# elizabethfong/SparkSmithWaterman

Hardware: AMD Instinct MI355X
Metric: GCUPS (higher is better)
Workload: dtype int32

## Files before the change

sparksmithwaterman_amd/csrc/swmi_api.cpp:

```cpp
#include <hip/hip_runtime.h>

#include <algorithm>
#include <atomic>
#include <chrono>
#include <condition_variable>
#include <unistd.h>
#include <cstdarg>
#include <cstdio>
#include <cstdlib>
#include <cstring>
#include <memory>
#include <mutex>
#include <numeric>
#include <string>
#include <thread>
#include <unordered_map>
#include <deque>
#include <vector>

#include "../../include/swmi.h"
#include "swmi_device.h"
#include "swmi_io_internal.h"

extern "C" hipError_t swmi_launch_fill(const FillArgs *a, hipStream_t st, hipEvent_t ev_start, hipEvent_t ev_stop);
extern "C" hipError_t swmi_launch_traceback(const TraceArgs *a, hipStream_t st, hipEvent_t ev_start, hipEvent_t ev_stop);
extern "C" hipError_t swmi_launch_traceback_split(const TraceArgs *a, uint32_t n_windows, hipStream_t st);
extern "C" hipError_t swmi_launch_resident(const TraceArgs *a, const ResidentArgs *x, hipStream_t st);
extern "C" hipError_t swmi_launch_tfused(const TraceArgs *a, const TFusedArgs *x, hipStream_t st);
extern "C" hipError_t swmi_launch_affine_sweep(const FillArgs *a, int32_t gap_open, uint32_t r_min, uint32_t r_max, hipStream_t st);
extern "C" hipError_t swmi_launch_affine_traceback(const TraceArgs *a, uint32_t tile_words, uint32_t ops_words, hipStream_t st);
extern "C" hipError_t swmi_launch_encode(const uint8_t *raw, const uint64_t *raw_off, SeqDesc *desc, uint32_t *seqw,
                                         const uint8_t *lut, uint32_t n_seq, hipStream_t st);

static thread_local std::string g_err;

static int fail(int code, const char *fmt, ...) {
    char buf[512];
    va_list ap;
    va_start(ap, fmt);
    vsnprintf(buf, sizeof buf, fmt, ap);
    va_end(ap);
    g_err = buf;
    return code;
}

int swmi_io_fail(int code, const std::string &msg) { return fail(code, "%s", msg.c_str()); }

#define HIP_TRY(expr)                                                                         \
    do {                                                                                      \
        hipError_t e_ = (expr);                                                               \
        if (e_ != hipSuccess)                                                                 \
            return fail(e_ == hipErrorOutOfMemory ? SWMI_ERR_NOMEM : SWMI_ERR_HIP,            \
                        "%s failed: %s", #expr, hipGetErrorString(e_));                       \
    } while (0)

struct DevBuf {
    void *p = nullptr;
    size_t cap = 0;
    int reserve(size_t bytes) {
        if (bytes <= cap) return SWMI_OK;
        size_t want = bytes >= (256u << 20) ? bytes + bytes / 2 : bytes;
        if (p) { want = std::max(want, cap + cap / 4); (void)hipFree(p); p = nullptr; cap = 0; }
        hipError_t e = hipMalloc(&p, want);
        if (e != hipSuccess && want > bytes) { want = bytes; e = hipMalloc(&p, want); }
        if (e != hipSuccess) { p = nullptr; return fail(SWMI_ERR_NOMEM, "hipMalloc(%zu) failed: %s", bytes, hipGetErrorString(e)); }
        cap = want;
        return SWMI_OK;
    }
    void release() { if (p) (void)hipFree(p); p = nullptr; cap = 0; }
    template <class T> T *as() const { return (T *)p; }
    DevBuf() = default;
    DevBuf(const DevBuf &) = delete;
    DevBuf &operator=(const DevBuf &) = delete;
    ~DevBuf() { release(); }
};

struct PinnedBuf {
    void *p = nullptr;
    void *dp = nullptr;
    size_t cap = 0;
    int reserve(size_t bytes) {
        if (bytes <= cap) return SWMI_OK;
        if (p) { bytes = std::max(bytes, cap + cap / 4); (void)hipHostFree(p); p = nullptr; dp = nullptr; cap = 0; }
        hipError_t e = hipHostMalloc(&p, bytes, hipHostMallocMapped);
        if (e != hipSuccess) { p = nullptr; return fail(SWMI_ERR_NOMEM, "hipHostMalloc(%zu) failed: %s", bytes, hipGetErrorString(e)); }
        e = hipHostGetDevicePointer(&dp, p, 0);
        if (e != hipSuccess) { (void)hipHostFree(p); p = nullptr; return fail(SWMI_ERR_HIP, "hipHostGetDevicePointer: %s", hipGetErrorString(e)); }
        cap = bytes;
        return SWMI_OK;
    }
    void release() { if (p) (void)hipHostFree(p); p = nullptr; dp = nullptr; cap = 0; }
    PinnedBuf() = default;
    PinnedBuf(const PinnedBuf &) = delete;
    PinnedBuf &operator=(const PinnedBuf &) = delete;
    ~PinnedBuf() { release(); }
};

struct swmi_ctx {
    int device = 0;
    hipStream_t stream = nullptr;
    std::mutex mu;
    uint32_t cell_cap = 64;
    uint64_t max_workspace_bytes = 32ull << 30;
    int profiling = 0;
    uint32_t mode = 1;
    int zero_copy = 1;
    uint64_t arena_words_per_pair = 160;
    uint64_t arena_copy_wpp = 160;
    uint64_t recs_per_pair_x16 = 32;
    hipEvent_t ev[6] = {nullptr, nullptr, nullptr, nullptr, nullptr, nullptr};
    PinnedBuf h_err;
    DevBuf d_hdr_ring;
    uint32_t hdr_next = 0;
    DevBuf d_lut;
    int64_t spin_us = 2000;
    uint32_t dbg_strip_spins = 0;
    uint32_t dbg_reverse_strips = 0;
    uint32_t auto_ties_x100 = 300;
    uint32_t col_chunks = 0;
    int tb_split = -1;
    bool ext_events = false;
    int tfused = -1;
    int resident = -1;
    int scores_only = 0;
    int stream_keep_records = 1;
    int device_strings = 1;
    bool cell_cap_set = false;
    int32_t gap_open = 0;
    int affine = -1;
    std::thread worker;
    std::mutex job_mu;
    std::condition_variable job_cv;
    std::atomic<int> job_state{0};
    swmi_batch *job_batch = nullptr;
    swmi_params job_params{};
    int job_rc = 0;
    std::string job_err;
};

struct HostAln {
    uint32_t rank;
    int32_t begin, end_i, end_j;
    uint32_t n_ops;
    const uint32_t *rec = nullptr;
    int64_t str_id = -1;
};

struct PairRes {
    int32_t score = 0;
    uint32_t flags = 0;
    uint64_t n_cells = 0;
    uint64_t first = 0;
    uint64_t count = 0;
};

struct SiteRef { uint64_t pair; uint64_t k; int32_t begin; };

struct Work {
    uint32_t pair;
    uint64_t cells;
    uint64_t dir_words;
    uint64_t seam_words;
};

struct swmi_batch {
    uint32_t n_refs = 0, n_reads = 0;
    std::vector<uint8_t> ref_bytes, read_bytes;
    const uint8_t *src_map = nullptr;
    std::vector<swmi_io_recpos> src_recs;
    std::unordered_map<uint32_t, std::vector<uint8_t>> src_cache;
    std::vector<uint64_t> ref_off, read_off;
    std::vector<SeqDesc> ref_desc, read_desc;
    DevBuf d_raw, d_raw_off;
    DevBuf d_seqw, d_refs, d_reads, d_pairs, d_dir, d_seam, d_result, d_cells, d_cells_off, d_cells_cap, d_dbg, d_dbg2;
    DevBuf d_strip_items, d_progress;
    DevBuf d_col_items;
    DevBuf d_win_off, d_queue;
    DevBuf d_tf_items;
    DevBuf d_res_items;
    bool views_built = false;
    bool tb_split_used = false;
    bool acgt_known = false;
    PinnedBuf h_result;
    swmi_params params{};
    bool has_run = false;
    int auto_choice = -1;
    swmi_params auto_params{};
    std::vector<Work> work;
    int work_mode = -1;
    bool work_tfused = false;
    uint32_t eff_mode = 1;
    int32_t gap_open = 0;
    uint64_t work_cells = 0;
    std::vector<uint8_t> pairs_on_device;
    const void *pairs_dev_ptr = nullptr;
    struct Prep {
        bool valid = false;
        size_t lo = 0, hi = 0;
        const void *work = nullptr;
        swmi_params params{};
        int mode = -1;
        uint64_t dir_words = 0, seam_words = 0;
        uint32_t max_path = 0, max_read = 0;
        size_t n_strip_items = 0, n_col_items = 0, n_strip_chunks = 0;
        uint64_t n_windows = 0, seam_priv_words = 0;
        size_t n_res = 0;
        uint32_t res_lds_words = 0, res_ops_words = 0;
        int resident_opt = -1;
        int tfused_opt = -1;
        uint32_t aff_r_min = 0, aff_r_max = 0;
        size_t n_tf = 0;
        uint32_t tf_max_m = 0, tf_max_n = 0, tf_max_path = 0;
        bool exact = false, scores_only = false;
        uint32_t col_chunks_opt = 0;
        bool reverse_strips = false;
    } prep;
    std::vector<PairRes> pairs;
    struct RawChunk { size_t at, words; size_t tab_at, n_rec; size_t lo; std::vector<uint32_t> wpos; };
    std::vector<uint32_t> raw;
    std::vector<AlnRec> rtab;
    const uint32_t *raw_ext = nullptr;
    const AlnRec *rtab_ext = nullptr;
    uint64_t raw_ext_records = 0, raw_ext_cap = 0;
    std::vector<RawChunk> raw_chunks;
    bool indexed = false;
    bool rec_strings = false;
    bool scores_only = false;
    bool records_dropped = false;
    std::vector<HostAln> alns;
    std::vector<char> str_buf;
    std::vector<uint64_t> str_at;
    std::vector<int8_t> ref_view_ready;
    std::vector<std::vector<SiteRef>> ref_sites;
    std::vector<uint64_t> ref_degenerate;
    swmi_timing timing{};
};

static const uint8_t *code_table();

extern "C" int swmi_abi_version(void) { return SWMI_ABI_VERSION; }

extern "C" const char *swmi_last_error(void) { return g_err.c_str(); }

extern "C" int swmi_device_count(int *count) {
    if (!count) return fail(SWMI_ERR_INVALID, "count is null");
    int n = 0;
    hipError_t e = hipGetDeviceCount(&n);
    if (e != hipSuccess) { *count = 0; return fail(SWMI_ERR_NO_DEVICE, "hipGetDeviceCount: %s", hipGetErrorString(e)); }
    *count = n;
    return SWMI_OK;
}

extern "C" void swmi_default_params(swmi_params *p) {
    if (!p) return;
    p->match = 5; p->mismatch = -3; p->gap = -4;
    p->tie_mode = SWMI_TIE_SERIAL;
    p->types[0] = 'a'; p->types[1] = 'i'; p->types[2] = 'd'; p->types[3] = '-';
}

static void ctx_release(swmi_ctx *c) {
    for (auto &ev : c->ev) if (ev) (void)hipEventDestroy(ev);
    if (c->stream) (void)hipStreamDestroy(c->stream);
    c->h_err.release();
    c->d_lut.release();
    c->d_hdr_ring.release();
    delete c;
}

extern "C" int swmi_create(int device, swmi_ctx **out) {
    if (!out) return fail(SWMI_ERR_INVALID, "out is null");
    *out = nullptr;
    int n = 0;
    hipError_t e = hipGetDeviceCount(&n);
    if (e != hipSuccess || n <= 0)
        return fail(SWMI_ERR_NO_DEVICE, "no HIP device available (%s); this library has no CPU fallback",
                    e != hipSuccess ? hipGetErrorString(e) : "device count 0");
    if (device < 0 || device >= n) return fail(SWMI_ERR_INVALID, "device %d out of range [0,%d)", device, n);
    hipDeviceProp_t prop;
    e = hipGetDeviceProperties(&prop, device);
    if (e != hipSuccess) return fail(SWMI_ERR_NO_DEVICE, "hipGetDeviceProperties: %s", hipGetErrorString(e));
    if (strncmp(prop.gcnArchName, "gfx950", 6) != 0)
        return fail(SWMI_ERR_NO_DEVICE, "device %d is %s; the kernels are built for gfx950 (MI355X) only",
                    device, prop.gcnArchName);
    e = hipSetDevice(device);
    if (e != hipSuccess) return fail(SWMI_ERR_NO_DEVICE, "hipSetDevice: %s", hipGetErrorString(e));
    swmi_ctx *c = new swmi_ctx;
    c->device = device;
    e = hipStreamCreateWithFlags(&c->stream, hipStreamNonBlocking);
    if (e != hipSuccess) { c->stream = nullptr; ctx_release(c); return fail(SWMI_ERR_HIP, "hipStreamCreate: %s", hipGetErrorString(e)); }
    for (auto &ev : c->ev) {
        e = hipEventCreate(&ev);
        if (e != hipSuccess) { ev = nullptr; ctx_release(c); return fail(SWMI_ERR_HIP, "hipEventCreate: %s", hipGetErrorString(e)); }
    }
    { int r = c->h_err.reserve(64); if (r) { ctx_release(c); return r; } }
    { static const char *ee = getenv("SWMI_EXT_EVENTS"); if (ee) c->ext_events = atoi(ee) != 0; }
// ... 50 lines not shown
        if (value < -1 || value > 1) return fail(SWMI_ERR_INVALID, "resident must be -1 (automatic), 0 or 1");
        ctx->resident = (int)value;
    } else if (!strcmp(name, "scores_only")) {
        ctx->scores_only = value != 0;
    } else if (!strcmp(name, "stream_keep_records")) {
        ctx->stream_keep_records = value != 0;
    } else if (!strcmp(name, "device_strings")) {
        ctx->device_strings = value != 0;
    } else if (!strcmp(name, "tb_split")) {
        if (value < -1 || value > 1) return fail(SWMI_ERR_INVALID, "tb_split must be -1 (automatic), 0 or 1");
        ctx->tb_split = (int)value;
    } else if (!strcmp(name, "col_chunks")) {
        if (value < 0 || value > 4096) return fail(SWMI_ERR_INVALID, "col_chunks out of range");
        ctx->col_chunks = (uint32_t)value;
    } else if (!strcmp(name, "zero_copy")) {
        ctx->zero_copy = value != 0;
    } else if (!strcmp(name, "profiling")) {
        if (value < 0 || value > 2) return fail(SWMI_ERR_INVALID, "profiling must be 0, 1 (every stage) or 2 (the sweep only)");
        ctx->profiling = (int)value;
    } else if (!strcmp(name, "gap_open")) {
        if (value > 0) return fail(SWMI_ERR_INVALID, "gap_open must be <= 0 (a penalty), got %lld", (long long)value);
        if (value < INT32_MIN) return fail(SWMI_ERR_INVALID, "gap_open out of range");
        ctx->gap_open = (int32_t)value;
    } else if (!strcmp(name, "affine")) {
        if (value != -1 && value != 1) return fail(SWMI_ERR_INVALID, "affine must be -1 (when gap_open != 0) or 1 (always)");
        ctx->affine = (int)value;
    } else if (!strcmp(name, "arena_words_per_pair")) {
        if (value < 1) return fail(SWMI_ERR_INVALID, "arena_words_per_pair out of range");
        ctx->arena_words_per_pair = (uint64_t)value;
    } else {
        return fail(SWMI_ERR_INVALID, "unknown option '%s'", name);
    }
    return SWMI_OK;
}

static const uint8_t *code_table() {
    static uint8_t T[256];
    static std::once_flag once;
    std::call_once(once, [] {
        uint8_t perm[256];
        for (int i = 0; i < 256; i++) perm[i] = (uint8_t)i;
        const uint8_t fast[8] = {'A', 'C', 'G', 'T', 'N', 'U', 'R', 'Y'};
        for (int k = 0; k < 8; k++) std::swap(perm[fast[k]], perm[4 * k]);
        for (int i = 0; i < 256; i++) {
            int u = i;
            if ((i >= 'a' && i <= 'z') || (i >= 0xE0 && i <= 0xFE && i != 0xF7)) u = i - 32;
            T[i] = perm[u];
        }
    });
    return T;
}

static uint64_t layout_sequences(const uint64_t *off, uint32_t n, uint64_t word0, std::vector<SeqDesc> &desc) {
    desc.resize(n);
    uint64_t at = word0;
    for (uint32_t s = 0; s < n; s++) {
        const uint64_t len = off[s + 1] - off[s];
        at = (at + 3) & ~(uint64_t)3;
        SeqDesc d{};
        d.len = (uint32_t)len;
        d.boff = (uint32_t)at;
        d.acgt = 0;
        desc[s] = d;
        at += (len + 3) / 4 + SWMI_SEQ_PAD_WORDS;
    }
    return at;
}

static int check_offsets(const uint64_t *off, uint32_t n, const char *what) {
    if (!off) return fail(SWMI_ERR_INVALID, "%s offsets are null", what);
    if (off[0] != 0) return fail(SWMI_ERR_INVALID, "%s offsets must start at 0", what);
    for (uint32_t k = 0; k < n; k++) {
        if (off[k + 1] < off[k]) return fail(SWMI_ERR_INVALID, "%s offsets decrease at %u", what, k);
        if (off[k + 1] - off[k] >= (1ull << 30))
            return fail(SWMI_ERR_UNSUPPORTED, "%s %u is longer than 2^30-1 bases", what, k);
    }
    return SWMI_OK;
}

extern "C" void swmi_batch_free(swmi_ctx *ctx, swmi_batch *b) {
    if (!b) return;
    if (ctx) (void)hipSetDevice(ctx->device);
    b->d_raw.release(); b->d_raw_off.release();
    b->d_seqw.release(); b->d_refs.release(); b->d_reads.release(); b->d_pairs.release();
    b->d_dir.release(); b->d_seam.release(); b->d_result.release(); b->d_cells.release();
    b->d_cells_off.release(); b->d_cells_cap.release(); b->d_dbg.release(); b->d_dbg2.release();
    b->d_strip_items.release(); b->d_progress.release(); b->d_col_items.release(); b->d_win_off.release(); b->d_queue.release(); b->d_res_items.release();
    b->d_tf_items.release();
    b->h_result.release();
    delete b;
}

static int upload_device(swmi_ctx *ctx, swmi_batch *b, hipStream_t st, const uint8_t *ref_src, const uint8_t *read_src) {
    const uint32_t n_refs = b->n_refs, n_reads = b->n_reads;
    const uint64_t ref_total = b->ref_off[n_refs], read_total = b->read_off[n_reads];
    uint64_t words = layout_sequences(b->ref_off.data(), n_refs, 0, b->ref_desc);
    words = layout_sequences(b->read_off.data(), n_reads, words, b->read_desc);
    words = ((words + 3) & ~(uint64_t)3) + SWMI_SEQ_PAD_WORDS;
    if (words >= (1ull << 32)) return fail(SWMI_ERR_UNSUPPORTED, "sequence image exceeds 16 GiB");
    int rc;
    const uint64_t read_base = (ref_total + 15) & ~(uint64_t)15;
    if ((rc = b->d_seqw.reserve(words * 4))) return rc;
    if ((rc = b->d_raw.reserve(read_base + read_total + 16))) return rc;
    if ((rc = b->d_raw_off.reserve(((uint64_t)n_refs + n_reads + 2) * 8))) return rc;
    if ((rc = b->d_refs.reserve(std::max<size_t>(n_refs, 1) * sizeof(SeqDesc)))) return rc;
    if ((rc = b->d_reads.reserve(std::max<size_t>(n_reads, 1) * sizeof(SeqDesc)))) return rc;
    HIP_TRY(hipMemsetAsync(b->d_seqw.p, 0, words * 4, st));
    uint8_t *raw = b->d_raw.as<uint8_t>();
    uint64_t *roff = b->d_raw_off.as<uint64_t>();
    if (ref_total) HIP_TRY(hipMemcpyAsync(raw, ref_src, ref_total, hipMemcpyHostToDevice, st));
    if (read_total) HIP_TRY(hipMemcpyAsync(raw + read_base, read_src, read_total, hipMemcpyHostToDevice, st));
    HIP_TRY(hipMemcpyAsync(roff, b->ref_off.data(), ((size_t)n_refs + 1) * 8, hipMemcpyHostToDevice, st));
    std::vector<uint64_t> read_abs(b->read_off);
    for (auto &o : read_abs) o += read_base;
    HIP_TRY(hipMemcpyAsync(roff + n_refs + 1, read_abs.data(), ((size_t)n_reads + 1) * 8, hipMemcpyHostToDevice, st));
    if (n_refs) HIP_TRY(hipMemcpyAsync(b->d_refs.p, b->ref_desc.data(), n_refs * sizeof(SeqDesc), hipMemcpyHostToDevice, st));
    if (n_reads) HIP_TRY(hipMemcpyAsync(b->d_reads.p, b->read_desc.data(), n_reads * sizeof(SeqDesc), hipMemcpyHostToDevice, st));
    HIP_TRY(swmi_launch_encode(raw, roff, b->d_refs.as<SeqDesc>(), b->d_seqw.as<uint32_t>(), ctx->d_lut.as<uint8_t>(), n_refs, st));
    HIP_TRY(swmi_launch_encode(raw, roff + n_refs + 1, b->d_reads.as<SeqDesc>(), b->d_seqw.as<uint32_t>(),
                               ctx->d_lut.as<uint8_t>(), n_reads, st));
    HIP_TRY(hipStreamSynchronize(st));
    b->work_mode = -1; b->prep.valid = false; b->pairs_dev_ptr = nullptr; b->pairs_on_device.clear();
    b->has_run = false; b->acgt_known = false; b->auto_choice = -1;
    return SWMI_OK;
}

extern "C" int swmi_batch_upload(swmi_ctx *ctx,
                                 const uint8_t *ref_bytes, const uint64_t *ref_off, uint32_t n_refs,
                                 const uint8_t *read_bytes, const uint64_t *read_off, uint32_t n_reads,
                                 swmi_batch **out) {
    if (!ctx || !out) return fail(SWMI_ERR_INVALID, "null argument");
    *out = nullptr;
    int rc;
    if ((rc = check_offsets(ref_off, n_refs, "reference"))) return rc;
    if ((rc = check_offsets(read_off, n_reads, "read"))) return rc;
    if ((n_refs && ref_off[n_refs] && !ref_bytes) || (n_reads && read_off[n_reads] && !read_bytes))
        return fail(SWMI_ERR_INVALID, "sequence bytes are null");
    if ((uint64_t)n_refs * n_reads >= (1ull << 32))
        return fail(SWMI_ERR_UNSUPPORTED, "more than 2^32-1 pairs in one batch");
    std::lock_guard<std::mutex> g(ctx->mu);
    HIP_TRY(hipSetDevice(ctx->device));

    std::unique_ptr<swmi_batch> b(new swmi_batch);
    b->n_refs = n_refs; b->n_reads = n_reads;
    b->ref_off.assign(ref_off, ref_off + n_refs + 1);
    b->read_off.assign(read_off, read_off + n_reads + 1);
    b->ref_bytes.assign(ref_bytes, ref_bytes + ref_off[n_refs]);
    b->read_bytes.assign(read_bytes, read_bytes + read_off[n_reads]);
    if ((rc = upload_device(ctx, b.get(), ctx->stream, ref_bytes, read_bytes))) { swmi_batch_free(ctx, b.release()); return rc; }
    *out = b.release();
    return SWMI_OK;
}

namespace {

struct RunState {
    swmi_ctx *ctx;
    swmi_batch *b;
    FillArgs fa{};
    TraceArgs ta{};
    float fill_ms = 0, tb_ms = 0, d2h_ms = 0;
    uint32_t launches = 0;
    double enqueue_us = 0, wait_us = 0, copyout_us = 0, prep_us = 0, prep_upload_us = 0;
    bool one_wave_sweep = false;
    bool tb_split = false;
    bool defer_copy = false;
    bool keep = true;
};

inline size_t result_out_off() { return 64; }
inline size_t result_tab_off(size_t np) { return (64 + np * sizeof(PairOut) + 255) & ~(size_t)255; }
inline size_t result_arena_off(size_t np, uint64_t tab_cap) { return (result_tab_off(np) + tab_cap * sizeof(AlnRec) + 255) & ~(size_t)255; }
inline uint64_t rec_words(uint32_t n_ops, bool strings) {
    return strings ? 2 * ((uint64_t)n_ops / 4 + 1) : ((uint64_t)n_ops + 15) / 16;
}

}

#define SWMI_RES_CELL_CAP 128u

static uint64_t path_bound(uint64_t n_, uint64_t m_, const swmi_params &p) {
    uint64_t path = n_ + m_;
    if (p.match > 0 && p.gap < 0 && p.mismatch <= p.match) {
        const uint64_t g = (uint64_t)(-(int64_t)p.gap), mt = (uint64_t)p.match;
        path = std::min(path, std::min(m_ + std::min(n_, mt * m_ / g), n_ + std::min(m_, mt * n_ / g)));
    }
    return path;
}

static uint64_t traceback_lds_bytes(uint32_t mode, uint64_t max_path, uint64_t max_read) {
    const uint64_t lds_words = (max_path + 3) / 4 + 1, lds_read_words = (max_read + 3) / 4 + 1;
    const uint64_t win = (uint64_t)SWMI_RMAX * 64;
    const uint64_t tile_words = mode == 0 ? 4ull * 16 * win : (mode == 1 ? 32 + 8ull * SWMI_CK_BLOCKS * win : 4ull * SWMI_CK_BLOCKS * win);
    return 4ull * (tile_words + 4ull * (lds_words + lds_read_words + 96));
}

static int prepare_chunk(RunState &rs, const std::vector<Work> &work, size_t lo, size_t hi, const std::vector<uint64_t> *cells_exact) {
    swmi_ctx *ctx = rs.ctx;
    swmi_batch *b = rs.b;
    const size_t np = hi - lo;
    const uint32_t n_reads = b->n_reads;
    int rc;

    std::vector<PairDesc> pd;
    std::vector<StripItem> strip_items;
    uint64_t seam_priv_words = 0;
    size_t n_strip_chunks = 0;
    std::vector<ColItem> col_items;
    uint64_t dir_words = 0, seam_words = 0;
    uint32_t max_path = 0, max_read = 0;
    size_t n_strip_items = 0, n_col_items = 0;
    uint64_t n_windows = 0;
    std::vector<uint32_t> win_off;
    std::vector<uint32_t> res_items;
    size_t n_res = 0;
    uint32_t res_lds_words = 0, res_ops_words = 0;
    std::vector<uint32_t> tf_items;
    size_t n_tf = 0;
    uint32_t tf_max_m = 0, tf_max_n = 0, tf_max_path = 0;
    uint32_t aff_r_min = 0xFFFFFFFFu, aff_r_max = 0;
    const uint32_t res_cell_cap = SWMI_RES_CELL_CAP;
    swmi_batch::Prep &pr = b->prep;
    const auto p0 = std::chrono::steady_clock::now();
    const bool prepared = pr.valid && pr.lo == lo && pr.hi == hi && pr.work == (const void *)work.data() && pr.mode == b->eff_mode &&
                          memcmp(&pr.params, &b->params, sizeof(swmi_params)) == 0 && b->pairs_dev_ptr == b->d_pairs.p &&
                          b->pairs_on_device.size() == np * sizeof(PairDesc) && pr.col_chunks_opt == ctx->col_chunks &&
                          pr.reverse_strips == (ctx->dbg_reverse_strips != 0) && pr.resident_opt == ctx->resident &&
                          pr.tfused_opt == ctx->tfused && pr.exact == (cells_exact != nullptr) && pr.scores_only == (ctx->scores_only != 0);
    if (prepared) {
        dir_words = pr.dir_words; seam_words = pr.seam_words; max_path = pr.max_path; max_read = pr.max_read;
        n_strip_items = pr.n_strip_items; n_col_items = pr.n_col_items; n_windows = pr.n_windows;
        seam_priv_words = pr.seam_priv_words; n_strip_chunks = pr.n_strip_chunks;
        n_res = pr.n_res; res_lds_words = pr.res_lds_words; res_ops_words = pr.res_ops_words;
        n_tf = pr.n_tf; tf_max_m = pr.tf_max_m; tf_max_n = pr.tf_max_n; tf_max_path = pr.tf_max_path;
        aff_r_min = pr.aff_r_min; aff_r_max = pr.aff_r_max;
    } else {
    const swmi_params &P = b->params;
    const bool cols_possible = b->eff_mode == 1 && P.match > 0 && P.gap < 0 && P.mismatch <= 0 &&
                               P.match <= 7 && P.mismatch >= -8 && (np <= 512 || ctx->col_chunks > 1) && ctx->col_chunks != 1;
    const bool res_possible = b->eff_mode == 1 && !cells_exact && !ctx->scores_only && ctx->resident != 0 && (ctx->resident == 1 || np >= 256) &&
                              P.match <= 7 && P.match >= -8 && P.mismatch >= -8 && P.mismatch <= 0 && P.gap <= 0;
    auto res_need_words = [&](uint32_t m_, uint32_t n_, uint32_t &opw) -> uint64_t {
        const uint32_t R_ = swmi_rows_per_lane(m_), lact = (m_ + R_ - 1) / R_;
        const uint64_t nblk = ((uint64_t)n_ + lact - 1 + 15) / 16, n_ck = (nblk + SWMI_CK_BLOCKS - 1) / SWMI_CK_BLOCKS;
        opw = (uint32_t)((path_bound(n_, m_, P) + 15) / 16 + 1);
        return nblk * R_ * 64 + ((n_ck + 1) & ~1ull) + 2ull * res_cell_cap + 64ull * opw + (n_ + 3) / 4 + 1 + (m_ + 3) / 4 + 1 + 8 +
               128;
    };
    bool res_maybe = false;
    if (res_possible)
        for (size_t k = 0; k < np && !res_maybe; k++) {
            const uint32_t m_ = b->read_desc[work[lo + k].pair % n_reads].len, n_ = b->ref_desc[work[lo + k].pair / n_reads].len;
            uint32_t opw;
            res_maybe = m_ <= 64u * SWMI_RMAX && (ctx->resident == 1 || (uint64_t)n_ <= 8ull * m_) &&
                        res_need_words(m_, n_, opw) * 4 <= (ctx->resident == 1 ? 40u : 20u) * 1024u;
        }
    const bool tf_possible = b->eff_mode == 1 && !cells_exact && !ctx->scores_only && ctx->tfused == 1 &&
                             P.match > 0 && P.match <= 7 && P.mismatch >= -8 && P.mismatch <= P.match && P.gap < 0 && P.gap >= -64;
    if ((cols_possible || res_maybe || tf_possible) && !b->acgt_known) {
        if (b->n_refs) HIP_TRY(hipMemcpy(b->ref_desc.data(), b->d_refs.p, b->n_refs * sizeof(SeqDesc), hipMemcpyDeviceToHost));
        if (b->n_reads) HIP_TRY(hipMemcpy(b->read_desc.data(), b->d_reads.p, b->n_reads * sizeof(SeqDesc), hipMemcpyDeviceToHost));
        b->acgt_known = true;
    }
    const uint64_t chunk_budget = ctx->col_chunks > 1 ? ctx->col_chunks : std::max<uint64_t>(1, 1024 / std::max<size_t>(np, 1));
    pd.resize(np);
    if (b->eff_mode == 1) win_off.resize(np + 1);
    uint32_t pb_m = 0xFFFFFFFFu, pb_n = 0xFFFFFFFFu, pb_val = 0;
    for (size_t k = 0; k < np; k++) {
        const Work &w = work[lo + k];
        PairDesc d{};
        d.ref_id = w.pair / n_reads;
        d.read_id = w.pair % n_reads;
        d.out_id = (uint32_t)k;
        const uint32_t m_ = b->read_desc[d.read_id].len, n_ = b->ref_desc[d.ref_id].len;
        if (b->eff_mode == 1) {
            const uint64_t rps = 64ull * swmi_rows_per_lane(m_);
            const uint64_t wb = ((uint64_t)n_ + 63u + 15u) / 16u;
            win_off[k] = (uint32_t)std::min<uint64_t>(n_windows, 0xFFFFFFFFu);
            n_windows += ((m_ + rps - 1) / rps) * ((wb + SWMI_CK_BLOCKS - 1u) / SWMI_CK_BLOCKS);
        }
        uint32_t res_opw = 0;
        const bool res_fit = res_maybe && m_ <= 64u * SWMI_RMAX && b->read_desc[d.read_id].acgt && b->ref_desc[d.ref_id].acgt &&
                             (ctx->resident == 1 || (uint64_t)n_ <= 8ull * m_) &&
                             res_need_words(m_, n_, res_opw) * 4 <= (ctx->resident == 1 ? 40u : 20u) * 1024u;
        const bool tf_fit = !res_fit && tf_possible && m_ <= SWMI_TF_MAX_M && n_ <= 64u * SWMI_TF_BMAX &&
                            b->read_desc[d.read_id].acgt && b->ref_desc[d.ref_id].acgt && w.dir_words >= swmi_tf_ck_words(m_);
        if (tf_fit) {
            d.pad = SWMI_PAD_RESIDENT;
            tf_items.push_back((uint32_t)k);
            tf_max_m = std::max(tf_max_m, m_); tf_max_n = std::max(tf_max_n, n_);
            tf_max_path = std::max<uint32_t>(tf_max_path, (uint32_t)path_bound(n_, m_, P));
        } else if (res_fit) {
            d.pad = SWMI_PAD_RESIDENT;
            res_items.push_back((uint32_t)k);
            uint32_t opw;
            res_lds_words = std::max<uint32_t>(res_lds_words, (uint32_t)res_need_words(m_, n_, opw));
            res_ops_words = std::max(res_ops_words, opw);
        } else if (b->eff_mode == 1 && m_ > 64u * SWMI_RMAX && strip_items.size() < (1u << 30)) {
            const uint32_t strips = (m_ + 64u * SWMI_RMAX - 1u) / (64u * SWMI_RMAX);
            d.pad = (uint32_t)strip_items.size();
            auto push_strips = [&](StripItem it) {
                it.pair = (uint32_t)k;
                it.prog = (uint32_t)strip_items.size();
                it.pad = 0;
                if (ctx->dbg_reverse_strips) for (uint32_t st = strips; st-- > 0;) { it.strip = st; strip_items.push_back(it); }
                else                         for (uint32_t st = 0; st < strips; st++) { it.strip = st; strip_items.push_back(it); }
            };
            uint64_t chunks = 1;
            const uint64_t wblocks = ((uint64_t)n_ + 63u + 15u) / 16u;
            const uint32_t n_ck = (uint32_t)((wblocks + SWMI_CK_BLOCKS - 1u) / SWMI_CK_BLOCKS);
            const uint32_t step_w = 16u * SWMI_CK_BLOCKS;
            const uint64_t span = (uint64_t)m_ + (uint64_t)(P.match > 0 ? P.match : 0) * m_ / (uint64_t)(P.gap < 0 ? -(int64_t)P.gap : 1) + 1;
            if (cols_possible) {
                const uint64_t budget = ctx->col_chunks > 1 ? ctx->col_chunks : chunk_budget / strips;
                chunks = std::min<uint64_t>(budget, n_ / std::max<uint64_t>((span + 64) / 4, 256));
                chunks = std::min<uint64_t>(chunks, n_ck);
                if (chunks < 2) chunks = 1;
            }
            if (chunks == 1) {
                StripItem it{};
                it.col0 = 0; it.g_lo = 0; it.g_hi = 0xFFFFFFFFu; it.priv_stride = 0; it.priv_off = 0;
                push_strips(it);
            } else {
                const uint32_t wpc = (uint32_t)((n_ck + chunks - 1) / chunks);
                for (uint32_t g_lo = 0; g_lo < n_ck; g_lo += wpc) {
                    StripItem it{};
                    it.g_lo = g_lo;
                    it.g_hi = std::min(g_lo + wpc, n_ck);
                    if (it.g_hi < n_ck && (uint64_t)it.g_hi * step_w > n_) it.g_hi = n_ck;
                    const int64_t c0 = (int64_t)g_lo * step_w - 64 - (int64_t)span - 1;
                    it.col0 = g_lo == 0 || c0 <= 0 ? 0u : (uint32_t)(c0 / step_w * step_w);
                    const uint64_t ext0 = (uint64_t)it.g_hi * step_w - it.col0 + 64ull * (strips - 1u);
                    const uint64_t n0 = it.g_hi < n_ck ? std::min<uint64_t>(n_ - it.col0, ext0) : n_ - it.col0;
                    it.priv_stride = (uint32_t)((n0 + 1 + 15) & ~15ull);
                    it.priv_off = seam_priv_words;
                    seam_priv_words += (uint64_t)(strips - 1u) * it.priv_stride;
                    if (it.g_hi == n_ck) it.g_hi = 0xFFFFFFFFu;
                    push_strips(it);
                    n_strip_chunks++;
                    if (it.g_hi == 0xFFFFFFFFu) break;
                }
            }
        } else if (cols_possible && chunk_budget > 1 && m_ <= 64u * SWMI_RMAX && b->read_desc[d.read_id].acgt && b->ref_desc[d.ref_id].acgt) {
            const uint64_t span = (uint64_t)m_ + (uint64_t)P.match * m_ / (uint64_t)(-(int64_t)P.gap) + 1;
            const uint64_t wblocks = ((uint64_t)n_ + 63u + 15u) / 16u;
            const uint32_t n_ck = (uint32_t)((wblocks + SWMI_CK_BLOCKS - 1u) / SWMI_CK_BLOCKS);
            const uint32_t step_w = 16u * SWMI_CK_BLOCKS;
            uint64_t chunks = std::min<uint64_t>(chunk_budget, n_ / std::max<uint64_t>(span + 64, 256));
            chunks = std::min<uint64_t>(chunks, n_ck);
            static const bool dbg_one = getenv("SWMI_DEBUG_ONE_CHUNK") != nullptr;
            if (dbg_one) chunks = 1;
            if (chunks >= 2 || dbg_one) {
                const uint32_t wpc = (uint32_t)((n_ck + chunks - 1) / chunks);
                const size_t first = col_items.size();
                for (uint32_t g_lo = 0; g_lo < n_ck; g_lo += wpc) {
                    ColItem ci;
                    ci.pair = (uint32_t)k;
                    ci.g_lo = g_lo;
                    ci.g_hi = std::min(g_lo + wpc, n_ck);
                    if (ci.g_hi < n_ck && (uint64_t)ci.g_hi * step_w > n_) ci.g_hi = n_ck;
                    const int64_t c0 = (int64_t)g_lo * step_w - 64 - (int64_t)span - 1;
                    ci.col0 = g_lo == 0 || c0 <= 0 ? 0u : (uint32_t)(c0 / step_w * step_w);
                    col_items.push_back(ci);
                    if (ci.g_hi == n_ck) break;
                }
                d.pad = SWMI_PAD_COLS | (uint32_t)(col_items.size() - first);
            }
        }
        pd[k] = d;
        if (m_ != pb_m || n_ != pb_n) { pb_m = m_; pb_n = n_; pb_val = (uint32_t)path_bound(n_, m_, b->params); }
        max_path = std::max<uint32_t>(max_path, pb_val);
        max_read = std::max(max_read, m_);
        aff_r_min = std::min(aff_r_min, swmi_aff_rows_per_lane(m_));
        aff_r_max = std::max(aff_r_max, swmi_aff_rows_per_lane(m_));
    }
    n_strip_items = strip_items.size();
    n_col_items = col_items.size();
    n_res = res_items.size();
    n_tf = tf_items.size();
    res_lds_words = 0;
    for (uint32_t k : res_items) {
        uint32_t opw;
        const uint32_t m_ = b->read_desc[pd[k].read_id].len, n_ = b->ref_desc[pd[k].ref_id].len;
        const uint64_t own = res_need_words(m_, n_, opw);
        res_lds_words = std::max<uint32_t>(res_lds_words, (uint32_t)(own + 64ull * (res_ops_words - opw)));
    }
    if (16ull * res_lds_words > 160ull * 1024) {
        for (uint32_t k : res_items) pd[k].pad = 0;
        res_items.clear();
        n_res = 0; res_lds_words = 0; res_ops_words = 0;
    }
    {
        std::vector<uint8_t> is_res(np, 0);
        for (uint32_t k : res_items) is_res[k] = 1;
        for (size_t k = 0; k < np; k++) {
            pd[k].dir_off = dir_words;
            pd[k].seam_off = seam_words;
            if (!is_res[k]) { dir_words += work[lo + k].dir_words; seam_words += work[lo + k].seam_words; }
        }
    }
    if (b->eff_mode == 1) win_off[np] = (uint32_t)std::min<uint64_t>(n_windows, 0xFFFFFFFFu);
    for (StripItem &it : strip_items)
        if (it.priv_stride) it.priv_off += seam_words;
    }
    const auto p1 = std::chrono::steady_clock::now();
    if (!prepared && b->eff_mode == 1) {
        if ((rc = b->d_win_off.reserve((np + 1) * sizeof(uint32_t)))) return rc;
        HIP_TRY(hipMemcpyAsync(b->d_win_off.p, win_off.data(), (np + 1) * sizeof(uint32_t), hipMemcpyHostToDevice, ctx->stream));
        HIP_TRY(hipStreamSynchronize(ctx->stream));
    }
    if ((rc = b->d_pairs.reserve(np * sizeof(PairDesc)))) return rc;
    if (!prepared && !strip_items.empty()) {
        if ((rc = b->d_strip_items.reserve(strip_items.size() * sizeof(StripItem)))) return rc;
        if ((rc = b->d_progress.reserve(strip_items.size() * sizeof(uint32_t)))) return rc;
        HIP_TRY(hipMemcpyAsync(b->d_strip_items.p, strip_items.data(), strip_items.size() * sizeof(StripItem), hipMemcpyHostToDevice, ctx->stream));
        HIP_TRY(hipStreamSynchronize(ctx->stream));
    }
    if (!prepared && !res_items.empty()) {
        if ((rc = b->d_res_items.reserve(res_items.size() * sizeof(uint32_t)))) return rc;
        HIP_TRY(hipMemcpyAsync(b->d_res_items.p, res_items.data(), res_items.size() * sizeof(uint32_t), hipMemcpyHostToDevice, ctx->stream));
        HIP_TRY(hipStreamSynchronize(ctx->stream));
    }
    if (!prepared && !tf_items.empty()) {
        if ((rc = b->d_tf_items.reserve(tf_items.size() * sizeof(uint32_t)))) return rc;
        HIP_TRY(hipMemcpyAsync(b->d_tf_items.p, tf_items.data(), tf_items.size() * sizeof(uint32_t), hipMemcpyHostToDevice, ctx->stream));
        HIP_TRY(hipStreamSynchronize(ctx->stream));
    }
    if (!prepared && !col_items.empty()) {
        if ((rc = b->d_col_items.reserve(col_items.size() * sizeof(ColItem)))) return rc;
        HIP_TRY(hipMemcpyAsync(b->d_col_items.p, col_items.data(), col_items.size() * sizeof(ColItem), hipMemcpyHostToDevice, ctx->stream));
        HIP_TRY(hipStreamSynchronize(ctx->stream));
    }
    if ((rc = b->d_dir.reserve(std::max<uint64_t>(dir_words, 1) * 4))) return rc;
    if ((rc = b->d_seam.reserve(std::max<uint64_t>(seam_words + seam_priv_words, 1) * 4))) return rc;
    if (!prepared && (b->pairs_dev_ptr != b->d_pairs.p || b->pairs_on_device.size() != np * sizeof(PairDesc) ||
        memcmp(b->pairs_on_device.data(), pd.data(), np * sizeof(PairDesc)) != 0)) {
        HIP_TRY(hipMemcpyAsync(b->d_pairs.p, pd.data(), np * sizeof(PairDesc), hipMemcpyHostToDevice, ctx->stream));
        HIP_TRY(hipStreamSynchronize(ctx->stream));
        b->pairs_on_device.assign((const uint8_t *)pd.data(), (const uint8_t *)pd.data() + np * sizeof(PairDesc));
        b->pairs_dev_ptr = b->d_pairs.p;
    }
    if (!prepared) {
        pr.valid = b->pairs_dev_ptr == b->d_pairs.p;
        pr.lo = lo; pr.hi = hi; pr.work = (const void *)work.data(); pr.params = b->params; pr.mode = b->eff_mode;
        pr.dir_words = dir_words; pr.seam_words = seam_words; pr.max_path = max_path; pr.max_read = max_read;
        pr.n_strip_items = n_strip_items; pr.n_col_items = n_col_items; pr.n_windows = n_windows;
        pr.seam_priv_words = seam_priv_words; pr.n_strip_chunks = n_strip_chunks;
        pr.n_res = n_res; pr.res_lds_words = res_lds_words; pr.res_ops_words = res_ops_words;
        pr.resident_opt = ctx->resident; pr.exact = cells_exact != nullptr;
        pr.tfused_opt = ctx->tfused; pr.n_tf = n_tf; pr.tf_max_m = tf_max_m; pr.tf_max_n = tf_max_n; pr.tf_max_path = tf_max_path;
        pr.col_chunks_opt = ctx->col_chunks; pr.reverse_strips = ctx->dbg_reverse_strips != 0;
        pr.scores_only = ctx->scores_only != 0;
        pr.aff_r_min = aff_r_min; pr.aff_r_max = aff_r_max;
    }
    rs.prep_us += std::chrono::duration<double, std::micro>(p1 - p0).count();
    rs.prep_upload_us += std::chrono::duration<double, std::micro>(std::chrono::steady_clock::now() - p1).count();
    return SWMI_OK;
}

static int dump_traceback_diagnostics(swmi_batch *b, const TraceArgs &ta, size_t np, size_t n_tf) {
    if (!ta.dbg) return SWMI_OK;
    std::vector<unsigned long long> d(np * 4);
    HIP_TRY(hipMemcpy(d.data(), ta.dbg, np * 32, hipMemcpyDeviceToHost));
    if (n_tf) {
        double t0 = 0, t1 = 0, t2 = 0, t3 = 0, t4 = 0, t5 = 0; unsigned long long mx = 0;
        for (size_t k = 0; k < np; k++) {
            t0 += d[4*k]; t1 += d[4*k+1] & 0xFFFFFFFFull; t2 += d[4*k+1] >> 32; t3 += d[4*k+2] >> 16; t4 += d[4*k+3] >> 32; t5 += d[4*k+3] & 0xFFFFFFFFull;
            mx = std::max(mx, d[4*k]);
        }
        fprintf(stderr, "[swmi tfused dbg] ticks per sweeper wavefront: lifetime mean=%.0f max=%llu = prologue %.0f + sweep %.0f + first block task %.0f (%.2f block tasks per wavefront) + waiting for tasks %.0f + rest (more tasks, walk items) %.0f\n",
                t0 / np, mx, t2 / np, t1 / np, t3 / np, t5 / np, t4 / np, (t0 - t1 - t2 - t3 - t4) / np);
        {
            std::vector<size_t> idx(np);
            for (size_t k = 0; k < np; k++) idx[k] = k;
            std::sort(idx.begin(), idx.end(), [&](size_t x, size_t y) { return d[4 * x] < d[4 * y]; });
            auto at = [&](double q) { return d[4 * idx[std::min<size_t>(np - 1, (size_t)(q * np))]]; };
            fprintf(stderr, "[swmi tfused dbg]   lifetime p10=%llu p50=%llu p90=%llu p99=%llu max=%llu\n", at(0.10), at(0.50), at(0.90), at(0.99), d[4 * idx[np - 1]]);
            for (size_t t = 0; t < std::min<size_t>(np, 6); t++) {
                const size_t k = idx[np - 1 - t];
                fprintf(stderr, "[swmi tfused dbg]   slow wavefront (pair %zu): lifetime %llu, sweep %llu, first block task %llu, block tasks taken %llu, waiting %llu, alignments of its pair %llu\n",
                        k, d[4 * k], d[4 * k + 1] & 0xFFFFFFFFull, d[4 * k + 2] >> 16, d[4 * k + 3] & 0xFFFFFFFFull, d[4 * k + 3] >> 32,
                        (unsigned long long)((const PairOut *)((const uint8_t *)b->h_result.p + result_out_off()))[k].n_cells);
            }
        }
    }
    double a0 = 0, a1 = 0, a2 = 0, a3 = 0; unsigned long long mx = 0;
    double a4 = 0;
    for (size_t k = 0; k < np; k++) { a0 += d[4*k]; a1 += d[4*k+1] & 0xFFFFFFFFull; a2 += d[4*k+2] & 0xFFFF; a4 += d[4*k+2] >> 16; a3 += d[4*k+3] & 0xFFFFFFFFull; mx = std::max(mx, d[4*k]); }
    fprintf(stderr, "[swmi tb dbg] wave ticks mean=%.0f max=%llu; walk ticks mean=%.0f; staging ticks mean=%.0f; steps mean=%.1f; iterations mean=%.2f\n",
            a0 / np, mx, a1 / np, a4 / np, a2 / np, a3 / np);
    const PairOut *po_dbg = (const PairOut *)((const uint8_t *)b->h_result.p + result_out_off());
    double cs[4] = {0, 0, 0, 0}, cw[4] = {0, 0, 0, 0}; unsigned long long cm[4] = {0, 0, 0, 0}; size_t cn[4] = {0, 0, 0, 0};
    for (size_t k = 0; k < np; k++) {
        const size_t c = std::min<uint64_t>(po_dbg[k].n_cells, 4) - (po_dbg[k].n_cells ? 1 : 0);
        cs[c] += d[4 * k]; cw[c] += d[4 * k + 1] & 0xFFFFFFFFull; cm[c] = std::max(cm[c], d[4 * k]); cn[c]++;
    }
    {
        std::vector<size_t> idx(np);
        for (size_t k = 0; k < np; k++) idx[k] = k;
        const size_t top = std::min<size_t>(np, 6);
        std::partial_sort(idx.begin(), idx.begin() + top, idx.end(), [&](size_t x, size_t y) { return d[4 * x] > d[4 * y]; });
        for (size_t t = 0; t < top; t++)
            fprintf(stderr, "[swmi tb dbg]   slow pair %zu: ticks=%llu walk=%llu staging=%llu in %llu stagings, steps=%llu iterations=%llu alignments=%llu\n", idx[t],
                    d[4 * idx[t]], d[4 * idx[t] + 1] & 0xFFFFFFFFull, d[4 * idx[t] + 2] >> 16, d[4 * idx[t] + 3] >> 32, d[4 * idx[t] + 2] & 0xFFFF,
                    d[4 * idx[t] + 3] & 0xFFFFFFFFull, (unsigned long long)po_dbg[idx[t]].n_cells);
        for (size_t t = 0; t < top; t++)
            fprintf(stderr, "[swmi tb dbg]     ... of the staging time of pair %zu, %llu ticks waiting for helpers\n", idx[t], d[4 * idx[t] + 1] >> 32);
    }
    for (int c = 0; c < 4; c++)
        if (cn[c]) fprintf(stderr, "[swmi tb dbg]   %d%s alignment(s): %zu pairs, wave ticks mean=%.0f max=%llu, walk(slot 0) mean=%.0f\n",
                           c + 1, c == 3 ? "+" : "", cn[c], cs[c] / cn[c], cm[c], cw[c] / cn[c]);
    return SWMI_OK;
}

static int dump_fill_diagnostics(swmi_batch *b, const FillArgs &fa, size_t np) {
    if (!fa.dbg) return SWMI_OK;
    std::vector<unsigned long long> d(np * 2);
    HIP_TRY(hipMemcpy(d.data(), fa.dbg, np * 16, hipMemcpyDeviceToHost));
#ifdef SWMI_STRIP_DIAG
    for (size_t k = 0; k < np && k < 8; k++)
        fprintf(stderr, "[swmi strip dbg] pair %zu: strip 0 lifetime %llu ticks, %llu waiting before publications; strip 1 lifetime %llu, "
                "%llu polls, %llu ticks in polls, %llu waiting for seam groups\n", k, d[2 * k] >> 32, d[2 * k] & 0xFFFFFFFFull,
                d[2 * k + 1] >> 40, (d[2 * k + 1] >> 32) & 0xFF, (d[2 * k + 1] >> 16) & 0xFFFF, d[2 * k + 1] & 0xFFFF);
#endif
    unsigned long long ev = 0, cyc = 0, evmax = 0, cmax = 0, cmin = ~0ull;
    for (size_t k = 0; k < np; k++) {
        ev += d[2 * k]; cyc += d[2 * k + 1];
        evmax = std::max(evmax, d[2 * k]); cmax = std::max(cmax, d[2 * k + 1]); cmin = std::min(cmin, d[2 * k + 1]);
    }
    fprintf(stderr, "[swmi fill dbg] pairs=%zu slow-path entries mean=%.1f max=%llu; wave ticks mean=%.0f min=%llu max=%llu\n",
            np, (double)ev / np, evmax, (double)cyc / np, cmin, cmax);
    if (b->eff_mode == 1) {
        std::unordered_map<unsigned long long, int> per_simd, per_cu;
        for (size_t k = 0; k < np; k++) {
            const unsigned long long hw = d[2 * k] & 0xFFFFFFFFull, xcc = (d[2 * k] >> 32) & 0xF;
            const unsigned long long simd = (hw >> 4) & 3, cu = (hw >> 8) & 15, sh = (hw >> 12) & 1, se = (hw >> 13) & 7;
// ... 12 lines not shown

static int keep_chunk_records(RunState &rs, const AlnRec *tab, uint64_t n_rec, const uint32_t *arena, uint64_t arena_cap, size_t lo) {
    swmi_batch *b = rs.b;
    if (rs.defer_copy && b->raw_chunks.empty()) {
        b->raw_ext = arena; b->rtab_ext = tab; b->raw_ext_records = n_rec; b->raw_ext_cap = arena_cap;
        b->raw_chunks.push_back(swmi_batch::RawChunk{0, 0, 0, (size_t)n_rec, lo, {}});
        return SWMI_OK;
    }
    uint64_t used = 0;
    for (uint64_t k = 0; k < n_rec; k++) {
        const uint64_t end = (((uint64_t)tab[k].off_hi << 32) | tab[k].off_lo) + rec_words(tab[k].n_ops, b->rec_strings);
        used = std::max(used, end);
    }
    if (used > arena_cap) return fail(SWMI_ERR_HIP, "record payloads overrun the arena");
    b->raw_chunks.push_back(swmi_batch::RawChunk{b->raw.size(), (size_t)used, b->rtab.size(), (size_t)n_rec, lo, {}});
    b->raw.insert(b->raw.end(), arena, arena + used);
    b->rtab.insert(b->rtab.end(), tab, tab + n_rec);
    return SWMI_OK;
}

static int run_chunk(RunState &rs, const std::vector<Work> &work, size_t lo, size_t hi,
                     const std::vector<uint64_t> *cells_exact, std::vector<PairOut> &outs) {
    swmi_ctx *ctx = rs.ctx;
    swmi_batch *b = rs.b;
    const size_t np = hi - lo;
    int rc;
    if ((rc = prepare_chunk(rs, work, lo, hi, cells_exact))) return rc;
    const swmi_batch::Prep &pr = b->prep;
    const uint64_t seam_words = pr.seam_words, n_windows = pr.n_windows;
    const uint32_t max_path = pr.max_path, max_read = pr.max_read;
    const size_t n_strip_items = pr.n_strip_items, n_col_items = pr.n_col_items, n_res = pr.n_res, n_tf = pr.n_tf;
    const uint32_t res_lds_words = pr.res_lds_words, res_ops_words = pr.res_ops_words, res_cell_cap = SWMI_RES_CELL_CAP;
    const uint32_t tf_max_m = pr.tf_max_m, tf_max_n = pr.tf_max_n, tf_max_path = pr.tf_max_path;
    if (seam_words) HIP_TRY(hipMemsetAsync(b->d_seam.p, 0, seam_words * 4, ctx->stream));

    uint32_t cell_cap = ctx->cell_cap;
    std::vector<uint64_t> coff;
    std::vector<uint32_t> ccap;
    uint64_t cells_total = 0;
    if (cells_exact) {
        coff.resize(np); ccap.resize(np);
        for (size_t k = 0; k < np; k++) {
            coff[k] = cells_total;
            ccap[k] = (uint32_t)std::min<uint64_t>((*cells_exact)[lo + k], 0xFFFFFFFFu);
            cells_total += ccap[k];
        }
        if ((rc = b->d_cells_off.reserve(np * 8))) return rc;
        if ((rc = b->d_cells_cap.reserve(np * 4))) return rc;
        HIP_TRY(hipMemcpyAsync(b->d_cells_off.p, coff.data(), np * 8, hipMemcpyHostToDevice, ctx->stream));
        HIP_TRY(hipMemcpyAsync(b->d_cells_cap.p, ccap.data(), np * 4, hipMemcpyHostToDevice, ctx->stream));
    } else {
        if (!ctx->cell_cap_set) cell_cap = (uint32_t)std::min<uint64_t>(65536, std::max<uint64_t>(cell_cap, (4ull << 20) / np));
        cells_total = (uint64_t)np * cell_cap;
    }
    if ((rc = b->d_cells.reserve(std::max<uint64_t>(cells_total, 1) * sizeof(uint2)))) return rc;

    const uint32_t lds_words = (max_path + 3) / 4 + 1;
    const uint32_t lds_read_words = (max_read + 3) / 4 + 1;
    {
        const uint64_t need = b->eff_mode == 3 ? 4ull * (SWMI_AFF_TILE_WORDS + ((uint64_t)max_path + 15) / 16 + 1 + 128)
                                               : traceback_lds_bytes(b->eff_mode, max_path, max_read);
        if (need > 160ull * 1024)
            return fail(SWMI_ERR_UNSUPPORTED, "a pair of %u bases in total needs %llu bytes of LDS for the traceback (limit 163840)",
                        max_path, (unsigned long long)need);
    }

    const auto c0 = std::chrono::steady_clock::now();
    uint64_t arena_cap = std::max<uint64_t>(np * ctx->arena_words_per_pair, 1024);
    uint64_t tab_cap = std::max<uint64_t>(np * ctx->recs_per_pair_x16 / 16 + 64, 256);
    std::vector<uint8_t> saved_outs;
    for (int attempt = 0;; attempt++) {
        if (attempt > 4) return fail(SWMI_ERR_HIP, "the record arena overflowed %d times in a row; results discarded", attempt);
        const size_t t_off = result_tab_off(np), a_off = result_arena_off(np, tab_cap);
        if ((rc = b->d_result.reserve(a_off + arena_cap * 4))) return rc;
        uint8_t *res = b->d_result.as<uint8_t>();
        if (attempt > 0) {
            HIP_TRY(hipMemsetAsync(res, 0, 64, ctx->stream));
            HIP_TRY(hipMemcpyAsync(res + result_out_off(), saved_outs.data(), saved_outs.size(),
                                   hipMemcpyHostToDevice, ctx->stream));
        }

        FillArgs &fa = rs.fa;
        fa.seqw = b->d_seqw.as<uint32_t>();
        fa.refs = b->d_refs.as<SeqDesc>();
        fa.reads = b->d_reads.as<SeqDesc>();
        fa.pairs = b->d_pairs.as<PairDesc>();
        fa.dir = b->d_dir.as<uint32_t>();
        fa.seam = b->d_seam.as<int32_t>();
        fa.out = (PairOut *)(res + result_out_off());
        fa.cells = b->d_cells.as<uint2>();
        fa.cells_off = cells_exact ? b->d_cells_off.as<uint64_t>() : nullptr;
        fa.cells_cap = cells_exact ? b->d_cells_cap.as<uint32_t>() : nullptr;
        fa.hdr = (ArenaHdr *)res;
        fa.dbg = nullptr;
        fa.dbg_pad = 0;
        static const bool dbg_fill = getenv("SWMI_DEBUG_FILL") != nullptr;
        if (dbg_fill) {
            if ((rc = b->d_dbg.reserve(np * 16))) return rc;
            fa.dbg = b->d_dbg.as<unsigned long long>();
            fa.dbg_thr0 = getenv("SWMI_DEBUG_THR0") ? (uint32_t)atoi(getenv("SWMI_DEBUG_THR0")) : 1u;
            fa.dbg_pad = getenv("SWMI_DEBUG_SKIP") ? 1u : 0u;
        }
        fa.n_pairs = (uint32_t)np;
        fa.cell_cap = cell_cap;
        fa.match = b->params.match; fa.mismatch = b->params.mismatch; fa.gap = b->params.gap;
        fa.strict = b->params.tie_mode == SWMI_TIE_STRICT;
        fa.mode = b->eff_mode;
        const bool pipe = n_strip_items && !rs.one_wave_sweep;
        fa.skip_multi = pipe ? 1u : 0u;
        fa.strip_items = pipe ? b->d_strip_items.as<StripItem>() : nullptr;
        fa.progress = pipe ? b->d_progress.as<uint32_t>() : nullptr;
        fa.n_strip_items = pipe ? (uint32_t)n_strip_items : 0u;
        fa.err_host = (uint32_t *)ctx->h_err.dp;
        fa.pad3 = 0;
        if (attempt == 0) b->timing.col_chunks += (uint32_t)n_col_items + (pipe ? (uint32_t)pr.n_strip_chunks : 0u);
        fa.col_items = n_col_items ? b->d_col_items.as<ColItem>() : nullptr;
        fa.n_col_items = (uint32_t)n_col_items;
        fa.strip_spins = ctx->dbg_strip_spins;
        const bool split_q = rs.tb_split && !cells_exact && b->eff_mode == 1 && n_windows < 0xFFFFFFFFull;
        const uint64_t q_cap = std::min<uint64_t>(std::max<uint64_t>(cells_total, 1), 1ull << 24);
        if (split_q && (rc = b->d_queue.reserve(256 + q_cap * sizeof(uint4)))) return rc;
        fa.q_reset = split_q ? b->d_queue.as<uint32_t>() : nullptr;

        TraceArgs &ta = rs.ta;
        ta.seqw = fa.seqw; ta.refs = fa.refs; ta.reads = fa.reads; ta.pairs = fa.pairs;
        ta.dir = fa.dir; ta.out = fa.out; ta.cells = fa.cells;
        ta.cells_off = fa.cells_off; ta.cells_cap = fa.cells_cap;
        ta.hdr = (ArenaHdr *)res;
        ta.arena = (uint32_t *)(res + a_off);
        ta.arena_cap_words = arena_cap;
        ta.rec_tab = (AlnRec *)(res + t_off);
        ta.rec_tab_cap = (uint32_t)std::min<uint64_t>(tab_cap, 0xFFFFFFFFu);
        ta.n_pairs = fa.n_pairs; ta.cell_cap = fa.cell_cap;
        ta.match = fa.match; ta.mismatch = fa.mismatch; ta.gap = fa.gap; ta.strict = fa.strict;
        ta.lds_words = lds_words;
        ta.seam = fa.seam;
        ta.mode = b->eff_mode;
        ta.pad2 = 0;
        ta.lds_read_words = lds_read_words;
        ta.out_host = nullptr;
        ta.ovf_host = (uint32_t *)ctx->h_err.dp + 4;
        ((volatile uint32_t *)ctx->h_err.p)[4] = 0u; ((volatile uint32_t *)ctx->h_err.p)[5] = 0u;
        ta.win_off = nullptr; ta.q_count = nullptr; ta.q_items = nullptr; ta.q_cap = 0; ta.pad4 = 0;
        const bool strings = ctx->device_strings != 0 && b->d_raw.p != nullptr;
        ta.raw = strings ? b->d_raw.as<uint8_t>() : nullptr;
        ta.raw_off = strings ? b->d_raw_off.as<uint64_t>() : nullptr;
        ta.raw_reads_at = b->n_refs + 1u;
        b->rec_strings = strings;
        ResidentArgs xa;
        xa.res_items = n_res ? b->d_res_items.as<uint32_t>() : nullptr;
        xa.n_res = (uint32_t)n_res; xa.res_lds_words = res_lds_words; xa.res_cell_cap = res_cell_cap; xa.res_ops_words = res_ops_words;
        TFusedArgs xt{};
        xt.items = n_tf ? b->d_tf_items.as<uint32_t>() : nullptr;
        xt.n_items = (uint32_t)n_tf;
        xt.cell_cap = 16;
        xt.tile_words = ((tf_max_m + 63u + 15u) / 16u) * 64u * SWMI_TF_BR;
        xt.ref_words = (tf_max_n + 3u) / 4u + 1u;
        xt.read_words = (tf_max_m + 3u) / 4u + 1u;
        xt.stage_words = (tf_max_path + 3u) / 4u + 1u + 128u;
        static const bool tf_marks = getenv("SWMI_DEBUG_MARKS") != nullptr;
        xt.debug_marks = tf_marks ? 1u : 0u;
        xt.lds_words = (xt.tile_words + 2u * xt.cell_cap + xt.stage_words + xt.ref_words + xt.read_words + 3u) & ~3u;
        {
            static const int tf_helpers = getenv("SWMI_TF_HELPERS") ? atoi(getenv("SWMI_TF_HELPERS")) : 2;
            const uint64_t region = 4ull * xt.lds_words, budget = 156ull * 1024;
            const uint64_t left = budget > 4 * region ? budget - 4 * region : 0;
            xt.n_helpers = (uint32_t)std::min<uint64_t>((uint64_t)std::max(0, std::min(tf_helpers, (int)SWMI_TF_HELPERS)), region ? left / region : 0);
        }
        const bool zc = ctx->zero_copy != 0;
        if (zc) {
            if ((rc = b->h_result.reserve(a_off + arena_cap * 4))) return rc;
            uint8_t *hd = (uint8_t *)b->h_result.dp;
            *(volatile uint32_t *)b->h_result.p = 0u;
            ((volatile uint32_t *)b->h_result.p)[1] = 0u;
            ta.ovf_host = (uint32_t *)hd;
            ta.out_host = (PairOut *)(hd + result_out_off());
            ta.arena = (uint32_t *)(hd + a_off);
            ta.rec_tab = (AlnRec *)(hd + t_off);
        }
        ta.dbg = nullptr;
        if (dbg_fill) {
            if ((rc = b->d_dbg2.reserve(np * 32))) return rc;
            HIP_TRY(hipMemsetAsync(b->d_dbg2.p, 0, np * 32, ctx->stream));
            ta.dbg = b->d_dbg2.as<unsigned long long>();
        }

        const bool whole_only = zc && n_tf + n_res == np;
        if (whole_only) {
            const uint32_t slots = 1024;
            if (!ctx->d_hdr_ring.p || ctx->hdr_next >= slots) {
                if ((rc = ctx->d_hdr_ring.reserve((size_t)slots * 64))) return rc;
                HIP_TRY(hipMemsetAsync(ctx->d_hdr_ring.p, 0, (size_t)slots * 64, ctx->stream));
                ctx->hdr_next = 0;
            }
            ta.hdr = (ArenaHdr *)(ctx->d_hdr_ring.as<uint8_t>() + (size_t)ctx->hdr_next++ * 64);
        }
        const bool split_now = rs.tb_split && !cells_exact && b->eff_mode == 1 && n_windows < 0xFFFFFFFFull;
// ... 1264 lines not shown
```

sparksmithwaterman_amd/csrc/swmi_device.h:

```cpp
#pragma once
#include <stdint.h>

#if defined(__HIPCC__)
#define SWMI_HD __host__ __device__
#else
#define SWMI_HD
#endif

#define SWMI_SEQ_PAD_WORDS 24u
#define SWMI_RMAX          4
#ifndef SWMI_CK_BLOCKS
#define SWMI_CK_BLOCKS     2u
#endif
#define SWMI_CODE_PAD      0x1FFu

#define SWMI_DIR_D 0u
#define SWMI_DIR_I 1u
#define SWMI_DIR_A 2u

#define SWMI_F_DEGENERATE   0x1u
#define SWMI_F_CELL_OVF     0x2u
#define SWMI_F_ARENA_OVF    0x4u
#define SWMI_F_DONE         0x8u

struct SeqDesc {
    uint32_t len;
    uint32_t boff;
    uint32_t acgt;
    uint32_t pad;
};

struct PairDesc {
    uint32_t ref_id;
    uint32_t read_id;
    uint32_t out_id;
    uint32_t pad;
    uint64_t dir_off;
    uint64_t seam_off;
};

#define SWMI_PAD_COLS 0x80000000u
#define SWMI_PAD_RESIDENT 0x40000000u

struct ColItem {
    uint32_t pair;
    uint32_t col0;
    uint32_t g_lo, g_hi;
};

struct StripItem {
    uint32_t pair, strip;
    uint32_t col0, g_lo, g_hi;
    uint32_t prog;
    uint32_t priv_stride;
    uint32_t pad;
    uint64_t priv_off;
};

struct PairOut {
    int32_t  score;
    uint32_t flags;
    uint64_t n_cells;
};

struct AlnRec {
    uint32_t out_id;
    uint32_t rank;
    int32_t  begin;
    int32_t  end_i, end_j;
    uint32_t n_ops;
    uint32_t off_lo, off_hi;
};
#define SWMI_RECTAB_WORDS 8u

struct ArenaHdr {
    unsigned long long reserved;
    unsigned long long pad;
};
#define SWMI_HDR_WORD_BITS 36u
#define SWMI_HDR_WORD_MASK ((1ull << SWMI_HDR_WORD_BITS) - 1ull)

struct FillArgs {
    const uint32_t *seqw;
    const SeqDesc  *refs;
    const SeqDesc  *reads;
    const PairDesc *pairs;
    uint32_t       *dir;
    int32_t        *seam;
    PairOut        *out;
    uint2          *cells;
    const uint64_t *cells_off;
    const uint32_t *cells_cap;
    ArenaHdr       *hdr;
    unsigned long long *dbg;
    uint32_t        dbg_thr0;
    uint32_t        dbg_pad;
    uint32_t        n_pairs;
    uint32_t        cell_cap;
    int32_t         match, mismatch, gap;
    uint32_t        strict;
    uint32_t        mode;
    uint32_t        skip_multi;
    const StripItem *strip_items;
    uint32_t       *progress;
    uint32_t        n_strip_items;
    uint32_t        pad3;
    uint32_t       *err_host;
    const ColItem  *col_items;
    uint32_t        n_col_items;
    uint32_t        strip_spins;
    uint32_t       *q_reset;
};

struct TraceArgs {
    const uint32_t *seqw;
    const SeqDesc  *refs;
    const SeqDesc  *reads;
    const PairDesc *pairs;
    const uint32_t *dir;
    PairOut        *out;
    const uint2    *cells;
    const uint64_t *cells_off;
    const uint32_t *cells_cap;
    ArenaHdr       *hdr;
    uint32_t       *arena;
    uint64_t        arena_cap_words;
    uint32_t        n_pairs;
    uint32_t        cell_cap;
    int32_t         match, mismatch, gap;
    uint32_t        strict;
    uint32_t        lds_words;
    uint32_t        lds_read_words;
    unsigned long long *dbg;
    const int32_t  *seam;
    PairOut        *out_host;
    uint32_t       *ovf_host;
    uint32_t        mode;
    uint32_t        pad2;
    const uint32_t *win_off;
    uint32_t       *q_count;
    uint4          *q_items;
    uint32_t        q_cap;
    uint32_t        pad4;
    const uint8_t  *raw;
    const uint64_t *raw_off;
    uint32_t        raw_reads_at;
    uint32_t        rec_tab_cap;
    AlnRec         *rec_tab;
};

struct ResidentArgs {
    const uint32_t *res_items;
    uint32_t        n_res;
    uint32_t        res_lds_words;
    uint32_t        res_cell_cap;
    uint32_t        res_ops_words;
};

struct TFusedArgs {
    const uint32_t *items;
    uint32_t        n_items;
    uint32_t        lds_words;
    uint32_t        tile_words;
    uint32_t        cell_cap;
    uint32_t        pad0;
    uint32_t        ref_words;
    uint32_t        read_words;
    uint32_t        stage_words;
    uint32_t        debug_marks;
    uint32_t        n_helpers;
};
#define SWMI_TF_HELPERS 2u
#define SWMI_TF_BMAX   40u
#ifndef SWMI_TF_BR
#define SWMI_TF_BR     4u
#endif
#define SWMI_TF_MAX_M  256u
SWMI_HD static inline uint32_t swmi_tf_cols_per_lane(uint32_t n) {
    uint32_t b = (n + 63u) / 64u;
    b = (b + 1u) & ~1u;
    return b < 2u ? 2u : b;
}
SWMI_HD static inline uint64_t swmi_tf_ck_words(uint32_t m) { return ((uint64_t)m + 64u) * 64u; }

#define SWMI_RANK_BY_CELL 0xFFFFFFFFu
#define SWMI_DETECT_LCAP  64u

SWMI_HD static inline uint32_t swmi_rows_per_lane(uint32_t m) {
    uint32_t r = (m + 63u) / 64u;
// ... 36 lines not shown
```

sparksmithwaterman_amd/csrc/swmi_kernels.hip:

```cpp
#include <hip/hip_runtime.h>
#include <hip/hip_ext.h>
#include <stdint.h>
#include <stdlib.h>
#include "swmi_device.h"
#include "swmi_emit.h"

#define WAVE 64
#ifndef SWMI_HELPER_SLEEP
#define SWMI_HELPER_SLEEP 8
#endif
#define BALLOT(pred) __builtin_amdgcn_ballot_w64(pred)
#define WAVE_SYNC() do { __builtin_amdgcn_fence(__ATOMIC_ACQ_REL, "wavefront"); __builtin_amdgcn_wave_barrier(); } while (0)

__device__ __forceinline__ int wave_shr1(int old, int src) {
    return __builtin_amdgcn_update_dpp(old, src, 0x138 , 0xf, 0xf, false);
}
__device__ __forceinline__ int wave_shr1_zero(int src) {
    return __builtin_amdgcn_update_dpp(0, src, 0x138 , 0xf, 0xf, true);
}

__device__ __forceinline__ int wave_max_i32(int v) {
#ifndef SWMI_NO_ASM
    asm volatile("s_nop 1\n\t"
                 "v_max_i32_dpp %0, %0, %0 row_shr:1 row_mask:0xf bank_mask:0xf\n\ts_nop 1\n\t"
// ... 478 lines not shown
            }
            if (reads_seam && (tb & 3u) == 0u) {
                SWMI_SD(const unsigned long long dg1 = __builtin_amdgcn_s_memtime();)
                seam_grp = seam_grp_next;
                SWMI_SD(asm volatile("s_waitcnt vmcnt(0)" : "+v"(seam_grp) :: "memory"); dg_grp += __builtin_amdgcn_s_memtime() - dg1;)
            }
            if (reads_seam && (tb & 3u) == 2u) seam_grp_next = load_group(tb / 4u + 1u);
            const int seamv = reads_seam ? __builtin_amdgcn_ds_bpermute((int)(((tb & 3u) << 6) + ((lane & 15u) << 2)), seam_grp) : 0;
            const bool steady = (t0 + 1u >= lact) && (t0 + 15u < n);
            uint32_t *pub_slot = PIPE ? progress + s : nullptr;
            const uint32_t pub_val = (PIPE && feeds_seam && tb > 0u && (tb % SWMI_PIPE_PUBLISH) == 0u) ? tb : 0u;
            if (steady)
                fill_block16<R, ACGT, STRICT, MULTI, false, MODE, PIPE>(S, w, t0, lane, lane_eff, n, m, row0, gap, match, mismatch,
                                                                        seamv, reads_seam, feeds_seam, seam_out, cells, ccap,
                                                                        pub_slot, pub_val, seam_sh, own_lo, own_hi);
            else
                fill_block16<R, ACGT, STRICT, MULTI, true, MODE, PIPE>(S, w, t0, lane, lane_eff, n, m, row0, gap, match, mismatch,
                                                                       seamv, reads_seam, feeds_seam, seam_out, cells, ccap,
                                                                       pub_slot, pub_val, seam_sh, own_lo, own_hi);
            if (PIPE && feeds_seam && tb + 1u == nblk) {
                asm volatile("s_waitcnt vmcnt(0)" ::: "memory");
                if (lane == 0) __hip_atomic_store(progress + s, nblk, __ATOMIC_RELAXED, __HIP_MEMORY_SCOPE_AGENT);
            }

            if (MODE == SWMI_MODE_FIELD) {
                const int miss = (int)(t0 + 15u) - ((int)(lane + n) - 1);
#pragma unroll
                for (int k = 0; k < R; ++k) {
                    uint32_t v = S.acc[k];
                    if (miss > 0 && miss < 16) v <<= 2 * miss;
                    wsp[((uint64_t)tb * R + k) * WAVE] = v;
                }
            }
        }
        if (MODE == SWMI_MODE_WINMAX) {
            const uint32_t gl = (nblk - 1u + (col0 >> 4)) / SWMI_CK_BLOCKS;
            if (gl >= g_lo && gl < g_hi) close_window(gl);
        }
#ifdef SWMI_STRIP_DIAG
        if (PIPE && A.dbg && lane == 0 && s < 2u) {
            const unsigned long long tot = __builtin_amdgcn_s_memtime() - t_start;
            A.dbg[2 * pd.out_id + s] = s == 0u ? (tot << 32) | (S.dg_pub & 0xFFFFFFFFull)
                                               : (tot << 40) | ((dg_polls & 0xFFull) << 32) | ((dg_poll & 0xFFFFull) << 16) | (dg_grp & 0xFFFFull);
        }
#endif
        if (S.ev_prev != 0) {
            handle_pending<R>(S, S.h, 16u * nblk - 1u, lane_eff, n, row0, m, cells, ccap);
            S.ev_prev = 0;
        }
        if (MULTI) __threadfence();
    }

    if (PIPE) {
        if (lane == 0 && pair_max > 0) atomicMax(&A.out[pd.out_id].score, pair_max);
        return;
    }
    if (lane == 0) {
        PairOut o;
        if (MODE == SWMI_MODE_WINMAX) {
            if (pair_max <= 0) { o.score = 0; o.flags = SWMI_F_DEGENERATE; o.n_cells = (uint64_t)m * n_full; }
            else               { o.score = pair_max; o.flags = 0u; o.n_cells = 0; }
        } else if (S.cnt == 0) { o.score = 0; o.flags = SWMI_F_DEGENERATE; o.n_cells = (uint64_t)m * n_full; }
        else            { o.score = S.thr; o.flags = S.cnt > ccap ? SWMI_F_CELL_OVF : 0u; o.n_cells = S.cnt; }
        A.out[pd.out_id] = o;
        if (A.dbg) {
            A.dbg[2 * pd.out_id] = S.events;
            A.dbg[2 * pd.out_id + 1] = __builtin_amdgcn_s_memtime() - t_start;
        }
    }
}

#include "swmi_step_gen.inc"

template <int R>
struct SweepState {
    int h[R], g[R];
    int hp[R];
    int q[R];
    int rbx, rby;
    int lmax;
};

template <int R>
__device__ __forceinline__ void sweep_step_ref(const int (&hin)[R], int (&hout)[R], int (&hp)[R], const int (&q)[R],
                                               const int rb, int &rbn, const uint32_t feed_code, const uint32_t gm,
                                               int &lm, const bool in_range) {
    const int nw = wave_shr1_zero(hout[R - 1]);
    const int upp = wave_shr1_zero(hp[R - 1]);
    if (in_range) {
        int diag = nw, up = upp;
#pragma unroll
        for (int k = 0; k < R; ++k) {
            const int a = __builtin_amdgcn_sdot8(q[k], rb, diag, false);
            diag = hin[k];
            int hv = a > up ? a : up;
            hv = hv > hp[k] ? hv : hp[k];
            hout[k] = hv;
            hp[k] = (uint32_t)hv > gm ? (int)((uint32_t)hv - gm) : 0;
            up = hp[k];
            lm = lm > hv ? lm : hv;
        }
    } else {
#pragma unroll
        for (int k = 0; k < R; ++k) hout[k] = hin[k];
    }
    rbn = wave_shr1((int)(1u << (feed_code & 31u)), rb);
}

template <int R>
__device__ __forceinline__ void sweep_tail_block(SweepState<R> &S, const uint4 w, const uint32_t wnext_x, const uint32_t t0,
                                                 const uint32_t lane_eff, const uint32_t n, const int one, const uint32_t gm) {
#ifndef SWMI_NO_ASM
    const uint32_t c = t0 - lane_eff;
    SweepStepTailAsm<R, 0>::run(S.h, S.g, S.hp, S.q, S.rbx, S.rby, w.x, w.y, one, gm, S.lmax, c + 0u, n);
    SweepStepTailAsm<R, 1>::run(S.h, S.g, S.hp, S.q, S.rbx, S.rby, w.x, w.y, one, gm, S.lmax, c + 1u, n);
    SweepStepTailAsm<R, 2>::run(S.h, S.g, S.hp, S.q, S.rbx, S.rby, w.x, w.y, one, gm, S.lmax, c + 2u, n);
    SweepStepTailAsm<R, 3>::run(S.h, S.g, S.hp, S.q, S.rbx, S.rby, w.x, w.y, one, gm, S.lmax, c + 3u, n);
    SweepStepTailAsm<R, 0>::run(S.h, S.g, S.hp, S.q, S.rbx, S.rby, w.y, w.z, one, gm, S.lmax, c + 4u, n);
    SweepStepTailAsm<R, 1>::run(S.h, S.g, S.hp, S.q, S.rbx, S.rby, w.y, w.z, one, gm, S.lmax, c + 5u, n);
    SweepStepTailAsm<R, 2>::run(S.h, S.g, S.hp, S.q, S.rbx, S.rby, w.y, w.z, one, gm, S.lmax, c + 6u, n);
    SweepStepTailAsm<R, 3>::run(S.h, S.g, S.hp, S.q, S.rbx, S.rby, w.y, w.z, one, gm, S.lmax, c + 7u, n);
    SweepStepTailAsm<R, 0>::run(S.h, S.g, S.hp, S.q, S.rbx, S.rby, w.z, w.w, one, gm, S.lmax, c + 8u, n);
    SweepStepTailAsm<R, 1>::run(S.h, S.g, S.hp, S.q, S.rbx, S.rby, w.z, w.w, one, gm, S.lmax, c + 9u, n);
    SweepStepTailAsm<R, 2>::run(S.h, S.g, S.hp, S.q, S.rbx, S.rby, w.z, w.w, one, gm, S.lmax, c + 10u, n);
    SweepStepTailAsm<R, 3>::run(S.h, S.g, S.hp, S.q, S.rbx, S.rby, w.z, w.w, one, gm, S.lmax, c + 11u, n);
    SweepStepTailAsm<R, 0>::run(S.h, S.g, S.hp, S.q, S.rbx, S.rby, w.w, wnext_x, one, gm, S.lmax, c + 12u, n);
    SweepStepTailAsm<R, 1>::run(S.h, S.g, S.hp, S.q, S.rbx, S.rby, w.w, wnext_x, one, gm, S.lmax, c + 13u, n);
    SweepStepTailAsm<R, 2>::run(S.h, S.g, S.hp, S.q, S.rbx, S.rby, w.w, wnext_x, one, gm, S.lmax, c + 14u, n);
    SweepStepTailAsm<R, 3>::run(S.h, S.g, S.hp, S.q, S.rbx, S.rby, w.w, wnext_x, one, gm, S.lmax, c + 15u, n);
#else
#pragma unroll
    for (uint32_t s = 0; s < 16; ++s) {
        const uint32_t s1 = s + 1u;
        const uint32_t wf = s1 < 4 ? w.x : s1 < 8 ? w.y : s1 < 12 ? w.z : s1 < 16 ? w.w : wnext_x;
        const uint32_t code = (wf >> (8u * (s1 & 3u))) & 0xFFu;
        const bool in_range = (t0 + s - lane_eff) < n;
        if (s & 1u) sweep_step_ref<R>(S.g, S.h, S.hp, S.q, S.rby, S.rbx, code, gm, S.lmax, in_range);
        else        sweep_step_ref<R>(S.h, S.g, S.hp, S.q, S.rbx, S.rby, code, gm, S.lmax, in_range);
    }
#endif
}

template <int R, bool COLS>
__device__ __forceinline__ void sweep_fast(const FillArgs &A, const PairDesc pd, const uint32_t lane, const ColItem ci) {
    const SeqDesc rd = A.refs[pd.ref_id];
    const SeqDesc qd = A.reads[pd.read_id];
    const uint32_t n_full = rd.len, m = qd.len;
    const StripGeom G = strip_geom<R>(m, n_full, 1u);
    const uint32_t col0 = COLS ? ci.col0 : 0u;
    const uint32_t g_lo = COLS ? ci.g_lo : 0u, g_hi = COLS ? ci.g_hi : G.n_ck;
    const bool last = g_hi >= G.n_ck;
    const uint32_t n = (last ? n_full : 16u * SWMI_CK_BLOCKS * g_hi) - col0;
    const uint32_t *__restrict__ refw = A.seqw + rd.boff + (col0 >> 2);
    const uint32_t *__restrict__ readw = A.seqw + qd.boff;
    const uint32_t lact = m >= G.rps ? WAVE : (m + R - 1) / R;
    const uint32_t lane_eff = lane < lact ? lane : 0x40000000u;
    const uint32_t T = n + lact - 1;
    const uint32_t nblk = last ? (T + 15u) / 16u : n / 16u;
    const uint32_t gm = (uint32_t)(-(int64_t)A.gap);
    const int one = 1;
    int pair_max = 0;

    const unsigned long long dbg_t0 = A.dbg ? __builtin_amdgcn_s_memtime() : 0ull;
    SweepState<R> S;
    build_profiles<R>(S.q, readw, lane * R, m, A.match, A.mismatch);
#pragma unroll
    for (int k = 0; k < R; ++k) {
        S.h[k] = 0; S.g[k] = 0; S.hp[k] = 0;
    }
    S.lmax = -1;
    const uint4 *__restrict__ refq = reinterpret_cast<const uint4 *>(refw);
    uint4 wnext = refq[0];
    S.rby = 0;
    S.rbx = wave_shr1((int)(1u << (wnext.x & 31u)), 0);

    uint32_t *__restrict__ wsp = A.dir + pd.dir_off + lane;
    auto close_window = [&](uint32_t g) {
        const int wm = wave_max_i32(lane < lact ? S.lmax : -1);
        if (lane == 0) A.dir[pd.dir_off + G.wmax_off + g] = (uint32_t)wm;
        pair_max = pair_max > wm ? pair_max : wm;
        S.lmax = -1;
    };
    for (uint32_t tb = 0; tb < nblk; ++tb) {
        const uint4 w = wnext;
        wnext = refq[tb + 1];
        const uint32_t tbg = tb + (col0 >> 4);
        if ((tbg % SWMI_CK_BLOCKS) == 0u) {
            const uint32_t g = tbg / SWMI_CK_BLOCKS;
            if (tb > 0u) {
                if (g > g_lo) close_window(g - 1u); else S.lmax = -1;
            }
            if (g >= g_lo) {
                uint32_t *__restrict__ ck = wsp + (uint64_t)g * (R + 2) * WAVE;
#pragma unroll
                for (int k = 0; k < R; ++k) ck[k * WAVE] = (uint32_t)S.h[k];
                ck[R * WAVE] = (uint32_t)wave_shr1_zero(S.g[R - 1]);
                ck[(R + 1) * WAVE] = (uint32_t)S.rby;
            }
        }
        const uint32_t t0 = 16u * tb;
#ifndef SWMI_NO_ASM
        if (t0 + 15u < n) {
            SweepStep4Asm<R>::run(S.h, S.g, S.hp, S.q, S.rbx, S.rby, w.x, w.y, one, gm, S.lmax);
            SweepStep4Asm<R>::run(S.h, S.g, S.hp, S.q, S.rbx, S.rby, w.y, w.z, one, gm, S.lmax);
            SweepStep4Asm<R>::run(S.h, S.g, S.hp, S.q, S.rbx, S.rby, w.z, w.w, one, gm, S.lmax);
            SweepStep4Asm<R>::run(S.h, S.g, S.hp, S.q, S.rbx, S.rby, w.w, wnext.x, one, gm, S.lmax);
        } else
#endif
        {
            sweep_tail_block<R>(S, w, wnext.x, t0, lane_eff, n, one, gm);
        }
    }
    {
        const uint32_t gl = (nblk - 1u + (col0 >> 4)) / SWMI_CK_BLOCKS;
        if (gl >= g_lo) close_window(gl);
    }
    if (lane != 0) return;
    if (A.dbg) {
        A.dbg[2 * pd.out_id] = (unsigned long long)__builtin_amdgcn_s_getreg((4 ) | (0 << 6) | (31 << 11)) |
                               ((unsigned long long)__builtin_amdgcn_s_getreg((20 ) | (0 << 6) | (31 << 11)) << 32);
        A.dbg[2 * pd.out_id + 1] = __builtin_amdgcn_s_memtime() - dbg_t0;
    }
    PairOut *o = &A.out[pd.out_id];
    if (COLS) {
        if (pair_max > 0) atomicMax(&o->score, pair_max);
        return;
    }
    PairOut v;
    if (pair_max <= 0) { v.score = 0; v.flags = SWMI_F_DEGENERATE; v.n_cells = (uint64_t)m * n_full; }
    else               { v.score = pair_max; v.flags = 0u; v.n_cells = 0; }
    *o = v;
}

template <bool COLS>
__device__ __forceinline__ void sweep_fast_dispatch(const FillArgs &A, const PairDesc pd, uint32_t lane, uint32_t m, const ColItem ci) {
    const uint32_t R = swmi_rows_per_lane(m);
    if (R == 1)      sweep_fast<1, COLS>(A, pd, lane, ci);
    else if (R == 2) sweep_fast<2, COLS>(A, pd, lane, ci);
    else if (R == 3) sweep_fast<3, COLS>(A, pd, lane, ci);
    else             sweep_fast<4, COLS>(A, pd, lane, ci);
}

template <bool ACGT, bool STRICT, int MODE>
__device__ __forceinline__ void fill_dispatch(const FillArgs &A, const PairDesc pd, uint32_t lane, uint32_t m) {
    const uint32_t R = swmi_rows_per_lane(m);
    if (R == 1)      fill_pair<1, ACGT, STRICT, false, MODE>(A, pd, lane);
    else if (R == 2) fill_pair<2, ACGT, STRICT, false, MODE>(A, pd, lane);
    else if (R == 3) fill_pair<3, ACGT, STRICT, false, MODE>(A, pd, lane);
    else if (m <= WAVE * SWMI_RMAX) fill_pair<SWMI_RMAX, ACGT, STRICT, false, MODE>(A, pd, lane);
    else             fill_pair<SWMI_RMAX, ACGT, STRICT, true, MODE>(A, pd, lane);
}

#define FILL_WAVES 4
template <int MODE>
__device__ __forceinline__ void fill_entry(const FillArgs &A) {
    const uint32_t pair = blockIdx.x * FILL_WAVES + (threadIdx.x >> 6);
    if (pair >= A.n_pairs) return;
    const uint32_t lane = threadIdx.x & 63u;
    if (pair == 0 && lane == 0 && A.hdr) { A.hdr->reserved = 0; A.hdr->pad = 0; }
    if (pair == 0 && lane == 0 && A.q_reset) *A.q_reset = 0u;
    const PairDesc pd = A.pairs[pair];
    if (MODE == SWMI_MODE_WINMAX && (pd.pad & SWMI_PAD_RESIDENT)) return;
    const SeqDesc rd = A.refs[pd.ref_id];
    const SeqDesc qd = A.reads[pd.read_id];
    if (MODE == SWMI_MODE_WINMAX && A.skip_multi && qd.len > WAVE * SWMI_RMAX) {
        if (lane == 0) { PairOut z; z.score = 0; z.flags = 0u; z.n_cells = 0; A.out[pd.out_id] = z; }
        return;
    }
    const bool acgt = rd.acgt && qd.acgt &&
                      SWMI_SCORES_FIT(A);
    if (MODE == SWMI_MODE_WINMAX && qd.len <= WAVE * SWMI_RMAX && (pd.pad & SWMI_PAD_COLS)) {
        if (lane == 0) { PairOut z; z.score = 0; z.flags = 0u; z.n_cells = 0; A.out[pd.out_id] = z; }
        return;
    }
    if (MODE == SWMI_MODE_WINMAX && acgt && qd.len <= WAVE * SWMI_RMAX && A.gap <= 0) {
        sweep_fast_dispatch<false>(A, pd, lane, qd.len, ColItem{0u, 0u, 0u, 0u});
        return;
    }
    if (MODE == SWMI_MODE_SCORE || MODE == SWMI_MODE_WINMAX) {
        if (acgt) fill_dispatch<true, false, MODE>(A, pd, lane, qd.len);
        else      fill_dispatch<false, false, MODE>(A, pd, lane, qd.len);
    } else if (acgt) {
        if (A.strict) fill_dispatch<true, true, MODE>(A, pd, lane, qd.len);
        else          fill_dispatch<true, false, MODE>(A, pd, lane, qd.len);
    } else {
        if (A.strict) fill_dispatch<false, true, MODE>(A, pd, lane, qd.len);
        else          fill_dispatch<false, false, MODE>(A, pd, lane, qd.len);
    }
}

extern "C" __global__ void __launch_bounds__(WAVE * FILL_WAVES)
sw_fill_kernel(const FillArgs A) { fill_entry<SWMI_MODE_FIELD>(A); }

extern "C" __global__ void __launch_bounds__(WAVE * FILL_WAVES)
sw_fill_score_kernel(const FillArgs A) { fill_entry<SWMI_MODE_SCORE>(A); }

extern "C" __global__ void __launch_bounds__(WAVE * FILL_WAVES) __attribute__((amdgpu_waves_per_eu(4, 4)))
sw_sweep_winmax_kernel(const FillArgs A) { fill_entry<SWMI_MODE_WINMAX>(A); }

extern "C" __global__ void __launch_bounds__(WAVE * FILL_WAVES)
sw_sweep_winmax_strips_kernel(const FillArgs A) {
    const uint32_t item = blockIdx.x * FILL_WAVES + (threadIdx.x >> 6);
    if (item >= A.n_strip_items) return;
    const uint32_t lane = threadIdx.x & 63u;
    const StripItem *it = A.strip_items + item;
    const PairDesc pd = A.pairs[it->pair];
    const SeqDesc rd = A.refs[pd.ref_id];
    const SeqDesc qd = A.reads[pd.read_id];
    const bool acgt = rd.acgt && qd.acgt &&
                      SWMI_SCORES_FIT(A);
    const uint32_t strip = __builtin_amdgcn_readfirstlane(it->strip);
    if (acgt) fill_pair<SWMI_RMAX, true, false, true, SWMI_MODE_WINMAX, true>(A, pd, lane, strip, it);
    else      fill_pair<SWMI_RMAX, false, false, true, SWMI_MODE_WINMAX, true>(A, pd, lane, strip, it);
}

extern "C" __global__ void __launch_bounds__(WAVE * FILL_WAVES)
sw_sweep_winmax_cols_kernel(const FillArgs A) {
    const uint32_t item = blockIdx.x * FILL_WAVES + (threadIdx.x >> 6);
    if (item >= A.n_col_items) return;
    const uint32_t lane = threadIdx.x & 63u;
    const ColItem ci = A.col_items[item];
    const PairDesc pd = A.pairs[ci.pair];
    sweep_fast_dispatch<true>(A, pd, lane, A.reads[pd.read_id].len, ci);
}

#define SWMI_TB_BLOCKS 16u
#define SWMI_TB_REFWIN_WORDS 96u
#define SWMI_TB_SLOTS 4u
#if SWMI_CK_BLOCKS > 2
#define SWMI_TB_WAVES 4u
#else
#define SWMI_TB_WAVES 8u
#endif

template <int R, bool STRICT>
__device__ __forceinline__ void replay_window_fast(const TraceArgs &A, const PairDesc pd, const uint32_t n, const uint32_t m,
                                                   const uint32_t *__restrict__ refw, const uint32_t *__restrict__ readw,
                                                   const uint32_t wlo, const uint32_t lane, uint32_t *__restrict__ lds_tile) {
    const uint32_t gm = (uint32_t)(-(int64_t)A.gap);
    const int one = 1;
    int h[R], g[R], hp[R], q[R];
    uint32_t acc[R];
    const uint32_t *__restrict__ ck = A.dir + pd.dir_off + (uint64_t)(wlo / SWMI_CK_BLOCKS) * (R + 2) * WAVE + lane;
    build_profiles<R>(q, readw, lane * R, m, A.match, A.mismatch);
#pragma unroll
    for (int k = 0; k < R; ++k) {
        h[k] = (int)ld_l2(ck + k * WAVE);
        hp[k] = (uint32_t)h[k] > gm ? (int)((uint32_t)h[k] - gm) : 0;
        g[k] = 0;
        acc[k] = 0;
    }
    const int nprev = (int)ld_l2(ck + R * WAVE);
    g[R - 1] = __builtin_amdgcn_update_dpp(0, nprev, 0x130 , 0xf, 0xf, true);
    const int rb_ck = (int)ld_l2(ck + (R + 1) * WAVE);
    const uint32_t lact = m >= WAVE * R ? WAVE : (m + R - 1) / R;
    const uint32_t T = n + lact - 1, nblk = (T + 15u) / 16u;
    const uint4 *__restrict__ refq = reinterpret_cast<const uint4 *>(refw);
    uint4 wv[SWMI_CK_BLOCKS + 1];
#pragma unroll
    for (uint32_t b = 0; b <= SWMI_CK_BLOCKS; ++b) wv[b] = refq[wlo + b];
    int rbx = wave_shr1((int)(1u << (wv[0].x & 31u)), rb_ck), rby = rb_ck;
#pragma unroll
    for (uint32_t b = 0; b < SWMI_CK_BLOCKS; ++b) {
        if (wlo + b >= nblk) break;
        const uint4 w = wv[b];
        DirStep4Asm<R, STRICT>::run(h, g, hp, acc, q, rbx, rby, w.x, w.y, one, gm);
        DirStep4Asm<R, STRICT>::run(h, g, hp, acc, q, rbx, rby, w.y, w.z, one, gm);
        DirStep4Asm<R, STRICT>::run(h, g, hp, acc, q, rbx, rby, w.z, w.w, one, gm);
        DirStep4Asm<R, STRICT>::run(h, g, hp, acc, q, rbx, rby, w.w, wv[b + 1].x, one, gm);
#pragma unroll
        for (int k = 0; k < R; ++k) lds_tile[(b * R + k) * WAVE + lane] = acc[k];
    }
}

template <int R, bool ACGT, bool STRICT, bool MULTI, bool DETECT>
__device__ __forceinline__ uint32_t replay_window(const TraceArgs &A, const PairDesc pd, const uint32_t n, const uint32_t m,
                                                  const uint32_t *__restrict__ refw, const uint32_t *__restrict__ readw,
                                                  const StripGeom G, const uint32_t s, const uint32_t wlo,
                                                  const uint32_t lane, uint32_t *__restrict__ lds_tile,
                                                  const int maxv, const uint32_t cnt_in, uint2 *__restrict__ cells, const uint32_t ccap) {
#ifndef SWMI_NO_ASM
// ... 1017 lines not shown
        if ((nops & 15u) != 0u && nops <= max_ops) my_ops[nops >> 4] = cur;
        WAVE_SYNC();
        const uint32_t opw = A.raw ? 0u : (nops + 15u) / 16u;
        const uint32_t words = mine ? swmi_payload_words(nops, A.raw != nullptr) : 0u;
        const uint32_t incl = wave_scan_add_u32(words);
        const uint32_t total = (uint32_t)__builtin_amdgcn_readlane((int)incl, 63);
        const uint32_t nhere = ncell - base < WAVE ? ncell - base : WAVE;
        unsigned long long off;
        uint32_t rslot;
        const bool fits = swmi_reserve(A, lane, total, nhere, off, rslot);
        const bool too_long = BALLOT(mine && nops > max_ops) != 0ull;
        if (fits && !too_long) {
            if (mine) {
                uint32_t *dst = A.arena + off + (incl - words);
                swmi_write_rec(A, rslot + lane, pd.out_id, SWMI_RANK_BY_CELL, begin, c0.x, c0.y, nops, off + (incl - words));
                for (uint32_t w = 0; w < opw; ++w) dst[w] = my_ops[w];
            }
            if (A.raw) {
                const uint8_t *__restrict__ raw_ref = A.raw + A.raw_off[pd.ref_id];
                const uint8_t *__restrict__ raw_read = A.raw + A.raw_off[A.raw_reads_at + pd.read_id];
                for (uint32_t a = 0; a < nhere; ++a) {
                    const uint32_t na = (uint32_t)__builtin_amdgcn_readlane((int)nops, (int)a);
                    const uint32_t at = (uint32_t)__builtin_amdgcn_readlane((int)(incl - words), (int)a);
                    const uint32_t ai = (uint32_t)__builtin_amdgcn_readlane((int)c0.x, (int)a);
                    const uint32_t aj = (uint32_t)__builtin_amdgcn_readlane((int)c0.y, (int)a);
                    swmi_emit_strings(A.arena + off + at, SwmiOpsPacked{opsb + a * X.res_ops_words},
                                      na, ai, aj, raw_ref, raw_read, lane, scratch);
                }
            }
        } else if (lane == 0) {
            atomicOr(&A.out[pd.out_id].flags, SWMI_F_ARENA_OVF);
            if (A.ovf_host) *A.ovf_host = 1u;
        }
        WAVE_SYNC();
    }
}

extern "C" __global__ void __launch_bounds__(WAVE * FILL_WAVES)
sw_resident_pairs_kernel(const TraceArgs A, const ResidentArgs X) {
    extern __shared__ uint32_t rp_lds[];
    const uint32_t wave = threadIdx.x >> 6, lane = threadIdx.x & 63u;
    const uint32_t item = blockIdx.x * FILL_WAVES + wave;
    if (item >= X.n_res) return;
    const PairDesc pd = A.pairs[X.res_items[item]];
    uint32_t *lds = rp_lds + wave * X.res_lds_words;
    const uint32_t R = swmi_rows_per_lane(A.reads[pd.read_id].len);
    if (A.strict) {
        if (R == 1)      resident_pair<1, true>(A, X, pd, lane, lds);
        else if (R == 2) resident_pair<2, true>(A, X, pd, lane, lds);
        else if (R == 3) resident_pair<3, true>(A, X, pd, lane, lds);
        else             resident_pair<4, true>(A, X, pd, lane, lds);
    } else {
        if (R == 1)      resident_pair<1, false>(A, X, pd, lane, lds);
        else if (R == 2) resident_pair<2, false>(A, X, pd, lane, lds);
        else if (R == 3) resident_pair<3, false>(A, X, pd, lane, lds);
        else             resident_pair<4, false>(A, X, pd, lane, lds);
    }
}

extern "C" hipError_t swmi_launch_resident(const TraceArgs *a, const ResidentArgs *x, hipStream_t st) {
    if (x->n_res == 0) return hipSuccess;
    static const bool attr = [] { (void)hipFuncSetAttribute(reinterpret_cast<const void *>(sw_resident_pairs_kernel),
                                                            hipFuncAttributeMaxDynamicSharedMemorySize, 160 * 1024); return true; }();
    (void)attr;
    hipLaunchKernelGGL(sw_resident_pairs_kernel, dim3((x->n_res + FILL_WAVES - 1) / FILL_WAVES), dim3(WAVE * FILL_WAVES),
                       (size_t)FILL_WAVES * x->res_lds_words * sizeof(uint32_t), st, *a, *x);
    return hipGetLastError();
}

static size_t spread_lds(uint32_t n_groups) {
    static const int on = getenv("SWMI_LDS_SPREAD") ? atoi(getenv("SWMI_LDS_SPREAD")) : 1;
    if (!on || n_groups == 0 || n_groups > 4u * 256u) return 0;
    const uint32_t per_cu = (n_groups + 255u) / 256u;
    return ((size_t)(160u * 1024u) / (per_cu + 1u) / 1024u + 1u) * 1024u;
}
template <class K>
static void allow_big_lds(K kernel) {
    (void)hipFuncSetAttribute(reinterpret_cast<const void *>(kernel), hipFuncAttributeMaxDynamicSharedMemorySize, 160 * 1024);
}

extern "C" hipError_t swmi_launch_fill(const FillArgs *a, hipStream_t st, hipEvent_t ev_start, hipEvent_t ev_stop) {
    if (a->n_pairs == 0) return hipSuccess;
    static const bool attrs = [] {
        allow_big_lds(sw_fill_kernel); allow_big_lds(sw_fill_score_kernel); allow_big_lds(sw_sweep_winmax_kernel);
        allow_big_lds(sw_sweep_winmax_strips_kernel); allow_big_lds(sw_sweep_winmax_cols_kernel);
        return true;
    }();
    (void)attrs;
    const dim3 grid((a->n_pairs + FILL_WAVES - 1) / FILL_WAVES), block(WAVE * FILL_WAVES);
    const size_t lds = spread_lds(grid.x);
    if (a->mode == 0)      hipLaunchKernelGGL(sw_fill_kernel, grid, block, lds, st, *a);
    else if (a->mode == 1) {
        if (ev_start && ev_stop && !(a->skip_multi && a->n_strip_items) && !a->n_col_items) {
            hipExtLaunchKernelGGL(sw_sweep_winmax_kernel, grid, block, (uint32_t)lds, st, ev_start, ev_stop, 0u, *a);
            return hipGetLastError();
        }
        hipLaunchKernelGGL(sw_sweep_winmax_kernel, grid, block, a->n_col_items || a->n_strip_items ? 0 : lds, st, *a);
        if (a->skip_multi && a->n_strip_items) {
            const uint32_t g = (a->n_strip_items + FILL_WAVES - 1) / FILL_WAVES;
            hipLaunchKernelGGL(sw_sweep_winmax_strips_kernel, dim3(g), block, spread_lds(g), st, *a);
        }
        if (a->n_col_items) {
            const uint32_t g = (a->n_col_items + FILL_WAVES - 1) / FILL_WAVES;
            hipLaunchKernelGGL(sw_sweep_winmax_cols_kernel, dim3(g), block, spread_lds(g), st, *a);
        }
    }
    else                   hipLaunchKernelGGL(sw_fill_score_kernel, grid, block, lds, st, *a);
    return hipGetLastError();
}

extern "C" hipError_t swmi_launch_traceback_split(const TraceArgs *a, uint32_t n_windows, hipStream_t st) {
    if (a->n_pairs == 0) return hipSuccess;
    const size_t win = (size_t)SWMI_CK_BLOCKS * SWMI_RMAX * WAVE;
    const size_t det_words = SWMI_SPLIT_WAVES * (win + 2u * SWMI_DETECT_LCAP);
    if (n_windows)
        hipLaunchKernelGGL(sw_detect_windows_kernel, dim3((n_windows + SWMI_SPLIT_WAVES - 1) / SWMI_SPLIT_WAVES), dim3(WAVE * SWMI_SPLIT_WAVES),
                           det_words * sizeof(uint32_t), st, *a);
    const size_t per_wave = (size_t)a->lds_words + a->lds_read_words + SWMI_TB_REFWIN_WORDS + win;
    uint32_t groups = (a->q_cap + SWMI_SPLIT_WAVES - 1) / SWMI_SPLIT_WAVES;
    if (groups > 2048u) groups = 2048u;
    if (groups < 1u) groups = 1u;
    hipLaunchKernelGGL(sw_walk_items_kernel, dim3(groups), dim3(WAVE * SWMI_SPLIT_WAVES), SWMI_SPLIT_WAVES * per_wave * sizeof(uint32_t), st, *a);
    return hipGetLastError();
}

extern "C" hipError_t swmi_launch_traceback(const TraceArgs *a, hipStream_t st, hipEvent_t ev_start, hipEvent_t ev_stop) {
    if (a->n_pairs == 0) return hipSuccess;
    const size_t tile = (size_t)(a->mode == 0 ? SWMI_TB_BLOCKS : SWMI_CK_BLOCKS) * SWMI_RMAX * WAVE;
    const size_t per_wave = (size_t)a->lds_words + a->lds_read_words + SWMI_TB_REFWIN_WORDS + tile;
    const dim3 block(WAVE * FILL_WAVES);
    if (a->mode == 1) {
        static int forced = getenv("SWMI_TB_WAVES") ? atoi(getenv("SWMI_TB_WAVES")) : 0;
        static int big = getenv("SWMI_TB_BIG") ? atoi(getenv("SWMI_TB_BIG")) : 10000;
        const uint32_t n_waves = forced ? (uint32_t)forced : (a->n_pairs <= 512u ? SWMI_TB_WAVES : a->n_pairs <= (uint32_t)big ? 4u : 1u);
        const size_t n_walkers = n_waves < SWMI_TB_SLOTS ? n_waves : SWMI_TB_SLOTS;
        const size_t tiles = (size_t)n_waves * SWMI_CK_BLOCKS * SWMI_RMAX * WAVE;
        size_t words = 32 + tiles + n_walkers * ((size_t)a->lds_words + a->lds_read_words + SWMI_TB_REFWIN_WORDS);
        static const int spec_opt = getenv("SWMI_TB_SPEC") ? atoi(getenv("SWMI_TB_SPEC")) : 1;
        TraceArgs t = *a;
        t.pad2 = (spec_opt && (spec_opt == 2 || a->n_pairs <= 384u) && n_waves > 1u && (words + tiles) * sizeof(uint32_t) <= 160u * 1024u) ? 1u : 0u;
        if (t.pad2) words += tiles;
        if (ev_start && ev_stop)
            hipExtLaunchKernelGGL(sw_traceback_winmax_kernel, dim3(a->n_pairs), dim3(WAVE * n_waves), (uint32_t)(words * sizeof(uint32_t)), st, ev_start, ev_stop, 0u, t);
        else
            hipLaunchKernelGGL(sw_traceback_winmax_kernel, dim3(a->n_pairs), dim3(WAVE * n_waves), words * sizeof(uint32_t), st, t);
    } else {
        const dim3 grid((a->n_pairs + FILL_WAVES - 1) / FILL_WAVES, SWMI_TB_SLOTS);
        if (a->mode == 0) hipLaunchKernelGGL(sw_traceback_kernel, grid, block, per_wave * FILL_WAVES * sizeof(uint32_t), st, *a);
        else              hipLaunchKernelGGL(sw_traceback_replay_kernel, grid, block, per_wave * FILL_WAVES * sizeof(uint32_t), st, *a);
    }
    return hipGetLastError();
}
```

sparksmithwaterman_amd/csrc/swmi_prep.hip:

```cpp
#include <hip/hip_runtime.h>
#include <stdint.h>
#include "swmi_device.h"

#define WAVE 64
#define ENC_WAVES 4

extern "C" __global__ void __launch_bounds__(WAVE * ENC_WAVES)
sw_encode_kernel(const uint8_t *__restrict__ raw, const uint64_t *__restrict__ raw_off, SeqDesc *__restrict__ desc,
                 uint32_t *__restrict__ seqw, const uint8_t *__restrict__ lut, uint32_t n_seq) {
    __shared__ uint8_t T[256];
    T[threadIdx.x] = lut[threadIdx.x];
    __syncthreads();
    const uint32_t s = blockIdx.x * ENC_WAVES + (threadIdx.x >> 6);
    if (s >= n_seq) return;
    const uint32_t lane = threadIdx.x & 63u;
    const uint64_t b0 = raw_off[s];
    const uint32_t len = (uint32_t)(raw_off[s + 1] - b0);
    uint32_t *__restrict__ img = seqw + desc[s].boff;
    const uint8_t *__restrict__ src = raw + b0;
    const uint32_t nw = (len + 3u) >> 2;
    uint32_t bad = 0;
    for (uint32_t w = lane; w < nw; w += WAVE) {
        const uint32_t k = 4u * w;
        uint32_t v = 0;
        const uint32_t c0 = T[src[k]];
        const uint32_t c1 = k + 1u < len ? T[src[k + 1u]] : 0u;
        const uint32_t c2 = k + 2u < len ? T[src[k + 2u]] : 0u;
        const uint32_t c3 = k + 3u < len ? T[src[k + 3u]] : 0u;
        v = c0 | (c1 << 8) | (c2 << 16) | (c3 << 24);
        bad |= v & 0xE3E3E3E3u;
        img[w] = v;
    }
    const uint64_t anybad = __builtin_amdgcn_ballot_w64(bad != 0u);
    if (lane == 0) desc[s].acgt = anybad ? 0u : 1u;
}

extern "C" hipError_t swmi_launch_encode(const uint8_t *raw, const uint64_t *raw_off, SeqDesc *desc, uint32_t *seqw,
                                         const uint8_t *lut, uint32_t n_seq, hipStream_t st) {
    if (n_seq == 0) return hipSuccess;
    hipLaunchKernelGGL(sw_encode_kernel, dim3((n_seq + ENC_WAVES - 1) / ENC_WAVES), dim3(WAVE * ENC_WAVES), 0, st,
                       raw, raw_off, desc, seqw, lut, n_seq);
    return hipGetLastError();
}
```

sparksmithwaterman_amd/csrc/swmi_step_gen.inc:

```
template <int R> struct SweepStep4Asm;

template <> struct SweepStep4Asm<1> {
    static __device__ __forceinline__ void run(int (&h)[1], int (&g)[1], int (&hp)[1], const int (&q)[1],
                                               int &rbx, int &rby, const uint32_t wf0, const uint32_t wf1,
                                               const int one, const uint32_t gm, int &lm) {
        int s0, a0, x;
        asm volatile(
            "v_dot8_i32_i4 %[s0], %[q0], %[rbx], 0\n\t"
            "v_lshlrev_b32_sdwa %[rby], %[wf0], %[one] dst_sel:DWORD dst_unused:UNUSED_PAD src0_sel:BYTE_1 src1_sel:DWORD\n\t"
            "v_max_i32_dpp %[x], %[p0], %[p0] wave_shr:1 row_mask:0xf bank_mask:0xf bound_ctrl:0\n\t"
            "s_nop 0\n\t"
            "v_add_u32_dpp %[a0], %[g0], %[s0] wave_shr:1 row_mask:0xf bank_mask:0xf bound_ctrl:0\n\t"
            "v_mov_b32_dpp %[rby], %[rbx] wave_shr:1 row_mask:0xf bank_mask:0xf\n\t"
            "v_max_i32_e32 %[g0], %[a0], %[x]\n\t"
            "v_sub_u32_e64 %[p0], %[g0], %[gm] clamp\n\t"
            "v_dot8_i32_i4 %[s0], %[q0], %[rby], 0\n\t"
            "v_lshlrev_b32_sdwa %[rbx], %[wf0], %[one] dst_sel:DWORD dst_unused:UNUSED_PAD src0_sel:BYTE_2 src1_sel:DWORD\n\t"
            "v_max_i32_dpp %[x], %[p0], %[p0] wave_shr:1 row_mask:0xf bank_mask:0xf bound_ctrl:0\n\t"
            "s_nop 0\n\t"
            "v_add_u32_dpp %[a0], %[h0], %[s0] wave_shr:1 row_mask:0xf bank_mask:0xf bound_ctrl:0\n\t"
            "v_mov_b32_dpp %[rbx], %[rby] wave_shr:1 row_mask:0xf bank_mask:0xf\n\t"
            "v_max_i32_e32 %[h0], %[a0], %[x]\n\t"
            "v_sub_u32_e64 %[p0], %[h0], %[gm] clamp\n\t"
            "v_max3_i32 %[lm], %[lm], %[g0], %[h0]\n\t"
// ... 592 lines not shown
            "v_max_i32_dpp %[x], %[p3], %[p0] wave_shr:1 row_mask:0xf bank_mask:0xf bound_ctrl:0\n\t"
            "v_add_u32_dpp %[a0], %[h3], %[s0] wave_shr:1 row_mask:0xf bank_mask:0xf bound_ctrl:0\n\t"
            "v_mov_b32_dpp %[rbx], %[rby] wave_shr:1 row_mask:0xf bank_mask:0xf\n\t"
            "v_max_i32_e32 %[h0], %[a0], %[x]\n\t"
            "v_sub_u32_e64 %[p0], %[h0], %[gm] clamp\n\t"
            "v_max3_i32 %[h1], %[g0], %[p0], %[p1]\n\t"
            "v_sub_u32_e64 %[p1], %[h1], %[gm] clamp\n\t"
            "v_max3_i32 %[h2], %[g1], %[p1], %[p2]\n\t"
            "v_sub_u32_e64 %[p2], %[h2], %[gm] clamp\n\t"
            "v_max3_i32 %[h3], %[g2], %[p2], %[p3]\n\t"
            "v_sub_u32_e64 %[p3], %[h3], %[gm] clamp\n\t"
            "v_max3_i32 %[x], %[lm], %[h0], %[h1]\n\t"
            "v_cndmask_b32_e32 %[lm], %[lm], %[x], vcc\n\t"
            "v_max3_i32 %[x], %[lm], %[h2], %[h3]\n\t"
            "v_cndmask_b32_e32 %[lm], %[lm], %[x], vcc\n\t"
            : [h0] "+v"(h[0]), [h1] "+v"(h[1]), [h2] "+v"(h[2]), [h3] "+v"(h[3]), [g0] "+v"(g[0]), [g1] "+v"(g[1]), [g2] "+v"(g[2]), [g3] "+v"(g[3]), [p0] "+v"(hp[0]), [p1] "+v"(hp[1]), [p2] "+v"(hp[2]), [p3] "+v"(hp[3]), [rbx] "+v"(rbx), [rby] "+v"(rby), [lm] "+v"(lm), [s0] "=&v"(s0), [a0] "=&v"(a0), [x] "=&v"(x), [a1] "=&v"(a1), [a2] "=&v"(a2), [a3] "=&v"(a3)
            : [q0] "v"(q[0]), [q1] "v"(q[1]), [q2] "v"(q[2]), [q3] "v"(q[3]), [wf0] "v"(wf0), [wf1] "v"(wf1), [one] "v"(one), [gm] "s"(gm), [c] "v"(c), [n] "v"(n)
            : "vcc");
    }
};

template <> struct SweepStepTailAsm<4, 2> {
    static __device__ __forceinline__ void run(int (&h)[4], int (&g)[4], int (&hp)[4], const int (&q)[4],
                                               int &rbx, int &rby, const uint32_t wf0, const uint32_t wf1,
                                               const int one, const uint32_t gm, int &lm, const uint32_t c, const uint32_t n) {
        int s0, a0, x, a1, a2, a3;
        asm volatile(
            "v_cmp_lt_u32_e32 vcc, %[c], %[n]\n\t"
            "v_dot8_i32_i4 %[s0], %[q0], %[rbx], 0\n\t"
            "v_dot8c_i32_i4_e32 %[h0], %[q1], %[rbx]\n\t"
            "v_dot8c_i32_i4_e32 %[h1], %[q2], %[rbx]\n\t"
            "v_dot8c_i32_i4_e32 %[h2], %[q3], %[rbx]\n\t"
            "v_lshlrev_b32_sdwa %[rby], %[wf0], %[one] dst_sel:DWORD dst_unused:UNUSED_PAD src0_sel:BYTE_3 src1_sel:DWORD\n\t"
            "v_max_i32_dpp %[x], %[p3], %[p0] wave_shr:1 row_mask:0xf bank_mask:0xf bound_ctrl:0\n\t"
            "v_add_u32_dpp %[a0], %[g3], %[s0] wave_shr:1 row_mask:0xf bank_mask:0xf bound_ctrl:0\n\t"
            "v_mov_b32_dpp %[rby], %[rbx] wave_shr:1 row_mask:0xf bank_mask:0xf\n\t"
            "v_max_i32_e32 %[g0], %[a0], %[x]\n\t"
            "v_sub_u32_e64 %[p0], %[g0], %[gm] clamp\n\t"
            "v_max3_i32 %[g1], %[h0], %[p0], %[p1]\n\t"
            "v_sub_u32_e64 %[p1], %[g1], %[gm] clamp\n\t"
            "v_max3_i32 %[g2], %[h1], %[p1], %[p2]\n\t"
            "v_sub_u32_e64 %[p2], %[g2], %[gm] clamp\n\t"
            "v_max3_i32 %[g3], %[h2], %[p2], %[p3]\n\t"
            "v_sub_u32_e64 %[p3], %[g3], %[gm] clamp\n\t"
            "v_max3_i32 %[x], %[lm], %[g0], %[g1]\n\t"
            "v_cndmask_b32_e32 %[lm], %[lm], %[x], vcc\n\t"
            "v_max3_i32 %[x], %[lm], %[g2], %[g3]\n\t"
            "v_cndmask_b32_e32 %[lm], %[lm], %[x], vcc\n\t"
            : [h0] "+v"(h[0]), [h1] "+v"(h[1]), [h2] "+v"(h[2]), [h3] "+v"(h[3]), [g0] "+v"(g[0]), [g1] "+v"(g[1]), [g2] "+v"(g[2]), [g3] "+v"(g[3]), [p0] "+v"(hp[0]), [p1] "+v"(hp[1]), [p2] "+v"(hp[2]), [p3] "+v"(hp[3]), [rbx] "+v"(rbx), [rby] "+v"(rby), [lm] "+v"(lm), [s0] "=&v"(s0), [a0] "=&v"(a0), [x] "=&v"(x), [a1] "=&v"(a1), [a2] "=&v"(a2), [a3] "=&v"(a3)
            : [q0] "v"(q[0]), [q1] "v"(q[1]), [q2] "v"(q[2]), [q3] "v"(q[3]), [wf0] "v"(wf0), [wf1] "v"(wf1), [one] "v"(one), [gm] "s"(gm), [c] "v"(c), [n] "v"(n)
            : "vcc");
    }
};

template <> struct SweepStepTailAsm<4, 3> {
    static __device__ __forceinline__ void run(int (&h)[4], int (&g)[4], int (&hp)[4], const int (&q)[4],
                                               int &rbx, int &rby, const uint32_t wf0, const uint32_t wf1,
                                               const int one, const uint32_t gm, int &lm, const uint32_t c, const uint32_t n) {
        int s0, a0, x, a1, a2, a3;
        asm volatile(
            "v_cmp_lt_u32_e32 vcc, %[c], %[n]\n\t"
            "v_dot8_i32_i4 %[s0], %[q0], %[rby], 0\n\t"
            "v_dot8c_i32_i4_e32 %[g0], %[q1], %[rby]\n\t"
            "v_dot8c_i32_i4_e32 %[g1], %[q2], %[rby]\n\t"
            "v_dot8c_i32_i4_e32 %[g2], %[q3], %[rby]\n\t"
            "v_lshlrev_b32_sdwa %[rbx], %[wf1], %[one] dst_sel:DWORD dst_unused:UNUSED_PAD src0_sel:BYTE_0 src1_sel:DWORD\n\t"
            "v_max_i32_dpp %[x], %[p3], %[p0] wave_shr:1 row_mask:0xf bank_mask:0xf bound_ctrl:0\n\t"
            "v_add_u32_dpp %[a0], %[h3], %[s0] wave_shr:1 row_mask:0xf bank_mask:0xf bound_ctrl:0\n\t"
            "v_mov_b32_dpp %[rbx], %[rby] wave_shr:1 row_mask:0xf bank_mask:0xf\n\t"
            "v_max_i32_e32 %[h0], %[a0], %[x]\n\t"
            "v_sub_u32_e64 %[p0], %[h0], %[gm] clamp\n\t"
            "v_max3_i32 %[h1], %[g0], %[p0], %[p1]\n\t"
            "v_sub_u32_e64 %[p1], %[h1], %[gm] clamp\n\t"
            "v_max3_i32 %[h2], %[g1], %[p1], %[p2]\n\t"
            "v_sub_u32_e64 %[p2], %[h2], %[gm] clamp\n\t"
            "v_max3_i32 %[h3], %[g2], %[p2], %[p3]\n\t"
            "v_sub_u32_e64 %[p3], %[h3], %[gm] clamp\n\t"
            "v_max3_i32 %[x], %[lm], %[h0], %[h1]\n\t"
            "v_cndmask_b32_e32 %[lm], %[lm], %[x], vcc\n\t"
            "v_max3_i32 %[x], %[lm], %[h2], %[h3]\n\t"
            "v_cndmask_b32_e32 %[lm], %[lm], %[x], vcc\n\t"
            : [h0] "+v"(h[0]), [h1] "+v"(h[1]), [h2] "+v"(h[2]), [h3] "+v"(h[3]), [g0] "+v"(g[0]), [g1] "+v"(g[1]), [g2] "+v"(g[2]), [g3] "+v"(g[3]), [p0] "+v"(hp[0]), [p1] "+v"(hp[1]), [p2] "+v"(hp[2]), [p3] "+v"(hp[3]), [rbx] "+v"(rbx), [rby] "+v"(rby), [lm] "+v"(lm), [s0] "=&v"(s0), [a0] "=&v"(a0), [x] "=&v"(x), [a1] "=&v"(a1), [a2] "=&v"(a2), [a3] "=&v"(a3)
            : [q0] "v"(q[0]), [q1] "v"(q[1]), [q2] "v"(q[2]), [q3] "v"(q[3]), [wf0] "v"(wf0), [wf1] "v"(wf1), [one] "v"(one), [gm] "s"(gm), [c] "v"(c), [n] "v"(n)
            : "vcc");
    }
};

template <int R, bool STRICT> struct DirStep4Asm;

template <> struct DirStep4Asm<1, false> {
    static __device__ __forceinline__ void run(int (&h)[1], int (&g)[1], int (&hp)[1], uint32_t (&acc)[1], const int (&q)[1],
                                               int &rbx, int &rby, const uint32_t wf0, const uint32_t wf1,
                                               const int one, const uint32_t gm) {
        int s0, a0, x;
        unsigned long long sI0, sA0, sI1, sA1;
        asm volatile(
            "v_dot8_i32_i4 %[s0], %[q0], %[rbx], 0\n\t"
            "v_lshlrev_b32_sdwa %[rby], %[wf0], %[one] dst_sel:DWORD dst_unused:UNUSED_PAD src0_sel:BYTE_1 src1_sel:DWORD\n\t"
            "v_mov_b32_dpp %[x], %[p0] wave_shr:1 row_mask:0xf bank_mask:0xf bound_ctrl:0\n\t"
            "s_nop 0\n\t"
            "v_add_u32_dpp %[a0], %[g0], %[s0] wave_shr:1 row_mask:0xf bank_mask:0xf bound_ctrl:0\n\t"
            "v_mov_b32_dpp %[rby], %[rbx] wave_shr:1 row_mask:0xf bank_mask:0xf\n\t"
            "v_cmp_ge_u32_e64 %[sI0], %[x], %[p0]\n\t"
            "v_max3_i32 %[g0], %[a0], %[x], %[p0]\n\t"
            "v_sub_u32_e64 %[p0], %[g0], %[gm] clamp\n\t"
            "v_cmp_eq_u32_e64 %[sA0], %[g0], %[a0]\n\t"
            "v_addc_co_u32_e64 %[c0], vcc, %[c0], %[c0], %[sI0]\n\t"
            "v_dot8_i32_i4 %[s0], %[q0], %[rby], 0\n\t"
            "v_addc_co_u32_e64 %[c0], vcc, %[c0], %[c0], %[sA0]\n\t"
            "v_lshlrev_b32_sdwa %[rbx], %[wf0], %[one] dst_sel:DWORD dst_unused:UNUSED_PAD src0_sel:BYTE_2 src1_sel:DWORD\n\t"
            "v_mov_b32_dpp %[x], %[p0] wave_shr:1 row_mask:0xf bank_mask:0xf bound_ctrl:0\n\t"
            "v_add_u32_dpp %[a0], %[h0], %[s0] wave_shr:1 row_mask:0xf bank_mask:0xf bound_ctrl:0\n\t"
            "v_mov_b32_dpp %[rbx], %[rby] wave_shr:1 row_mask:0xf bank_mask:0xf\n\t"
            "v_cmp_ge_u32_e64 %[sI0], %[x], %[p0]\n\t"
            "v_max3_i32 %[h0], %[a0], %[x], %[p0]\n\t"
            "v_sub_u32_e64 %[p0], %[h0], %[gm] clamp\n\t"
            "v_cmp_eq_u32_e64 %[sA0], %[h0], %[a0]\n\t"
            "v_addc_co_u32_e64 %[c0], vcc, %[c0], %[c0], %[sI0]\n\t"
            "v_dot8_i32_i4 %[s0], %[q0], %[rbx], 0\n\t"
            "v_addc_co_u32_e64 %[c0], vcc, %[c0], %[c0], %[sA0]\n\t"
            "v_lshlrev_b32_sdwa %[rby], %[wf0], %[one] dst_sel:DWORD dst_unused:UNUSED_PAD src0_sel:BYTE_3 src1_sel:DWORD\n\t"
            "v_mov_b32_dpp %[x], %[p0] wave_shr:1 row_mask:0xf bank_mask:0xf bound_ctrl:0\n\t"
            "v_add_u32_dpp %[a0], %[g0], %[s0] wave_shr:1 row_mask:0xf bank_mask:0xf bound_ctrl:0\n\t"
            "v_mov_b32_dpp %[rby], %[rbx] wave_shr:1 row_mask:0xf bank_mask:0xf\n\t"
            "v_cmp_ge_u32_e64 %[sI0], %[x], %[p0]\n\t"
            "v_max3_i32 %[g0], %[a0], %[x], %[p0]\n\t"
            "v_sub_u32_e64 %[p0], %[g0], %[gm] clamp\n\t"
            "v_cmp_eq_u32_e64 %[sA0], %[g0], %[a0]\n\t"
            "v_addc_co_u32_e64 %[c0], vcc, %[c0], %[c0], %[sI0]\n\t"
            "v_dot8_i32_i4 %[s0], %[q0], %[rby], 0\n\t"
            "v_addc_co_u32_e64 %[c0], vcc, %[c0], %[c0], %[sA0]\n\t"
            "v_lshlrev_b32_sdwa %[rbx], %[wf1], %[one] dst_sel:DWORD dst_unused:UNUSED_PAD src0_sel:BYTE_0 src1_sel:DWORD\n\t"
            "v_mov_b32_dpp %[x], %[p0] wave_shr:1 row_mask:0xf bank_mask:0xf bound_ctrl:0\n\t"
            "v_add_u32_dpp %[a0], %[h0], %[s0] wave_shr:1 row_mask:0xf bank_mask:0xf bound_ctrl:0\n\t"
            "v_mov_b32_dpp %[rbx], %[rby] wave_shr:1 row_mask:0xf bank_mask:0xf\n\t"
            "v_cmp_ge_u32_e64 %[sI0], %[x], %[p0]\n\t"
            "v_max3_i32 %[h0], %[a0], %[x], %[p0]\n\t"
            "v_sub_u32_e64 %[p0], %[h0], %[gm] clamp\n\t"
            "v_cmp_eq_u32_e64 %[sA0], %[h0], %[a0]\n\t"
            "v_addc_co_u32_e64 %[c0], vcc, %[c0], %[c0], %[sI0]\n\t"
            "s_nop 0\n\t"
            "v_addc_co_u32_e64 %[c0], vcc, %[c0], %[c0], %[sA0]\n\t"
            : [h0] "+v"(h[0]), [g0] "+v"(g[0]), [p0] "+v"(hp[0]), [c0] "+v"(acc[0]), [rbx] "+v"(rbx), [rby] "+v"(rby), [s0] "=&v"(s0), [a0] "=&v"(a0), [x] "=&v"(x), [sI0] "=&s"(sI0), [sA0] "=&s"(sA0), [sI1] "=&s"(sI1), [sA1] "=&s"(sA1)
            : [q0] "v"(q[0]), [wf0] "v"(wf0), [wf1] "v"(wf1), [one] "v"(one), [gm] "s"(gm)
            : "vcc");
    }
};

template <> struct DirStep4Asm<1, true> {
    static __device__ __forceinline__ void run(int (&h)[1], int (&g)[1], int (&hp)[1], uint32_t (&acc)[1], const int (&q)[1],
                                               int &rbx, int &rby, const uint32_t wf0, const uint32_t wf1,
                                               const int one, const uint32_t gm) {
        int s0, a0, x, t;
        unsigned long long sI0, sA0, sI1, sA1;
        asm volatile(
            "v_dot8_i32_i4 %[s0], %[q0], %[rbx], 0\n\t"
            "v_lshlrev_b32_sdwa %[rby], %[wf0], %[one] dst_sel:DWORD dst_unused:UNUSED_PAD src0_sel:BYTE_1 src1_sel:DWORD\n\t"
            "v_mov_b32_dpp %[x], %[p0] wave_shr:1 row_mask:0xf bank_mask:0xf bound_ctrl:0\n\t"
            "s_nop 0\n\t"
            "v_add_u32_dpp %[a0], %[g0], %[s0] wave_shr:1 row_mask:0xf bank_mask:0xf bound_ctrl:0\n\t"
            "v_mov_b32_dpp %[rby], %[rbx] wave_shr:1 row_mask:0xf bank_mask:0xf\n\t"
            "v_cmp_gt_u32_e64 %[sI0], %[x], %[p0]\n\t"
            "v_max_u32_e32 %[t], %[x], %[p0]\n\t"
            "v_max3_i32 %[g0], %[a0], %[x], %[p0]\n\t"
            "v_sub_u32_e64 %[p0], %[g0], %[gm] clamp\n\t"
            "v_cmp_gt_i32_e64 %[sA0], %[a0], %[t]\n\t"
// ... 765 lines not shown
```

Measured before the change: 2410.

## Precompute per-lane one-hot reference stream and add dedicated fast sweep kernel

```diff
diff --git a/sparksmithwaterman_amd/csrc/swmi_api.cpp b/sparksmithwaterman_amd/csrc/swmi_api.cpp
--- a/sparksmithwaterman_amd/csrc/swmi_api.cpp
+++ b/sparksmithwaterman_amd/csrc/swmi_api.cpp
@@ -30,7 +30,7 @@
 extern "C" hipError_t swmi_launch_affine_sweep(const FillArgs *a, int32_t gap_open, uint32_t r_min, uint32_t r_max, hipStream_t st);
 extern "C" hipError_t swmi_launch_affine_traceback(const TraceArgs *a, uint32_t tile_words, uint32_t ops_words, hipStream_t st);
 extern "C" hipError_t swmi_launch_encode(const uint8_t *raw, const uint64_t *raw_off, SeqDesc *desc, uint32_t *seqw,
-                                         const uint8_t *lut, uint32_t n_seq, hipStream_t st);
+                                         uint32_t *ohw, const uint8_t *lut, uint32_t n_seq, hipStream_t st);
 
 static thread_local std::string g_err;
 
@@ -172,6 +172,7 @@
     std::vector<uint64_t> ref_off, read_off;
     std::vector<SeqDesc> ref_desc, read_desc;
     DevBuf d_raw, d_raw_off;
+    DevBuf d_ohw;
     DevBuf d_seqw, d_refs, d_reads, d_pairs, d_dir, d_seam, d_result, d_cells, d_cells_off, d_cells_cap, d_dbg, d_dbg2;
     DevBuf d_strip_items, d_progress;
     DevBuf d_col_items;
@@ -211,6 +212,7 @@
         uint32_t aff_r_min = 0, aff_r_max = 0;
         size_t n_tf = 0;
         uint32_t tf_max_m = 0, tf_max_n = 0, tf_max_path = 0;
+        bool all_fast = false;
         bool exact = false, scores_only = false;
         uint32_t col_chunks_opt = 0;
         bool reverse_strips = false;
@@ -427,7 +429,7 @@
     if (!b) return;
     if (ctx) (void)hipSetDevice(ctx->device);
     b->d_raw.release(); b->d_raw_off.release();
-    b->d_seqw.release(); b->d_refs.release(); b->d_reads.release(); b->d_pairs.release();
+    b->d_seqw.release(); b->d_ohw.release(); b->d_refs.release(); b->d_reads.release(); b->d_pairs.release();
     b->d_dir.release(); b->d_seam.release(); b->d_result.release(); b->d_cells.release();
     b->d_cells_off.release(); b->d_cells_cap.release(); b->d_dbg.release(); b->d_dbg2.release();
     b->d_strip_items.release(); b->d_progress.release(); b->d_col_items.release(); b->d_win_off.release(); b->d_queue.release(); b->d_res_items.release();
@@ -446,11 +448,14 @@
     int rc;
     const uint64_t read_base = (ref_total + 15) & ~(uint64_t)15;
     if ((rc = b->d_seqw.reserve(words * 4))) return rc;
+    const uint64_t oh_words = SWMI_OH_FRONT + 4 * words;
+    if ((rc = b->d_ohw.reserve(oh_words * 4))) return rc;
     if ((rc = b->d_raw.reserve(read_base + read_total + 16))) return rc;
     if ((rc = b->d_raw_off.reserve(((uint64_t)n_refs + n_reads + 2) * 8))) return rc;
     if ((rc = b->d_refs.reserve(std::max<size_t>(n_refs, 1) * sizeof(SeqDesc)))) return rc;
     if ((rc = b->d_reads.reserve(std::max<size_t>(n_reads, 1) * sizeof(SeqDesc)))) return rc;
     HIP_TRY(hipMemsetAsync(b->d_seqw.p, 0, words * 4, st));
+    HIP_TRY(hipMemsetAsync(b->d_ohw.p, 0, oh_words * 4, st));
     uint8_t *raw = b->d_raw.as<uint8_t>();
     uint64_t *roff = b->d_raw_off.as<uint64_t>();
     if (ref_total) HIP_TRY(hipMemcpyAsync(raw, ref_src, ref_total, hipMemcpyHostToDevice, st));
@@ -461,8 +466,9 @@
     HIP_TRY(hipMemcpyAsync(roff + n_refs + 1, read_abs.data(), ((size_t)n_reads + 1) * 8, hipMemcpyHostToDevice, st));
     if (n_refs) HIP_TRY(hipMemcpyAsync(b->d_refs.p, b->ref_desc.data(), n_refs * sizeof(SeqDesc), hipMemcpyHostToDevice, st));
     if (n_reads) HIP_TRY(hipMemcpyAsync(b->d_reads.p, b->read_desc.data(), n_reads * sizeof(SeqDesc), hipMemcpyHostToDevice, st));
-    HIP_TRY(swmi_launch_encode(raw, roff, b->d_refs.as<SeqDesc>(), b->d_seqw.as<uint32_t>(), ctx->d_lut.as<uint8_t>(), n_refs, st));
-    HIP_TRY(swmi_launch_encode(raw, roff + n_refs + 1, b->d_reads.as<SeqDesc>(), b->d_seqw.as<uint32_t>(),
+    HIP_TRY(swmi_launch_encode(raw, roff, b->d_refs.as<SeqDesc>(), b->d_seqw.as<uint32_t>(), b->d_ohw.as<uint32_t>(),
+                               ctx->d_lut.as<uint8_t>(), n_refs, st));
+    HIP_TRY(swmi_launch_encode(raw, roff + n_refs + 1, b->d_reads.as<SeqDesc>(), b->d_seqw.as<uint32_t>(), b->d_ohw.as<uint32_t>(),
                                ctx->d_lut.as<uint8_t>(), n_reads, st));
     HIP_TRY(hipStreamSynchronize(st));
     b->work_mode = -1; b->prep.valid = false; b->pairs_dev_ptr = nullptr; b->pairs_on_device.clear();
@@ -564,6 +570,7 @@
     size_t n_tf = 0;
     uint32_t tf_max_m = 0, tf_max_n = 0, tf_max_path = 0;
     uint32_t aff_r_min = 0xFFFFFFFFu, aff_r_max = 0;
+    bool all_fast = false;
     const uint32_t res_cell_cap = SWMI_RES_CELL_CAP;
     swmi_batch::Prep &pr = b->prep;
     const auto p0 = std::chrono::steady_clock::now();
@@ -579,6 +586,7 @@
         n_res = pr.n_res; res_lds_words = pr.res_lds_words; res_ops_words = pr.res_ops_words;
         n_tf = pr.n_tf; tf_max_m = pr.tf_max_m; tf_max_n = pr.tf_max_n; tf_max_path = pr.tf_max_path;
         aff_r_min = pr.aff_r_min; aff_r_max = pr.aff_r_max;
+        all_fast = pr.all_fast;
     } else {
     const swmi_params &P = b->params;
     const bool cols_possible = b->eff_mode == 1 && P.match > 0 && P.gap < 0 && P.mismatch <= 0 &&
@@ -602,7 +610,9 @@
         }
     const bool tf_possible = b->eff_mode == 1 && !cells_exact && !ctx->scores_only && ctx->tfused == 1 &&
                              P.match > 0 && P.match <= 7 && P.mismatch >= -8 && P.mismatch <= P.match && P.gap < 0 && P.gap >= -64;
-    if ((cols_possible || res_maybe || tf_possible) && !b->acgt_known) {
+    const bool fast_possible = b->eff_mode == 1 && P.gap <= 0 && P.match >= -8 && P.match <= 7 && P.mismatch >= -8 && P.mismatch <= 7;
+    all_fast = fast_possible && np > 0;
+    if ((cols_possible || res_maybe || tf_possible || fast_possible) && !b->acgt_known) {
         if (b->n_refs) HIP_TRY(hipMemcpy(b->ref_desc.data(), b->d_refs.p, b->n_refs * sizeof(SeqDesc), hipMemcpyDeviceToHost));
         if (b->n_reads) HIP_TRY(hipMemcpy(b->read_desc.data(), b->d_reads.p, b->n_reads * sizeof(SeqDesc), hipMemcpyDeviceToHost));
         b->acgt_known = true;
@@ -713,6 +723,7 @@
             }
         }
         pd[k] = d;
+        all_fast = all_fast && d.pad == 0 && m_ <= 64u * SWMI_RMAX && b->read_desc[d.read_id].acgt && b->ref_desc[d.ref_id].acgt;
         if (m_ != pb_m || n_ != pb_n) { pb_m = m_; pb_n = n_; pb_val = (uint32_t)path_bound(n_, m_, b->params); }
         max_path = std::max<uint32_t>(max_path, pb_val);
         max_read = std::max(max_read, m_);
@@ -797,6 +808,7 @@
         pr.col_chunks_opt = ctx->col_chunks; pr.reverse_strips = ctx->dbg_reverse_strips != 0;
         pr.scores_only = ctx->scores_only != 0;
         pr.aff_r_min = aff_r_min; pr.aff_r_max = aff_r_max;
+        pr.all_fast = all_fast;
     }
     rs.prep_us += std::chrono::duration<double, std::micro>(p1 - p0).count();
     rs.prep_upload_us += std::chrono::duration<double, std::micro>(std::chrono::steady_clock::now() - p1).count();
@@ -975,6 +987,7 @@
 
         FillArgs &fa = rs.fa;
         fa.seqw = b->d_seqw.as<uint32_t>();
+        fa.ohw = b->d_ohw.as<uint32_t>();
         fa.refs = b->d_refs.as<SeqDesc>();
         fa.reads = b->d_reads.as<SeqDesc>();
         fa.pairs = b->d_pairs.as<PairDesc>();
@@ -1005,7 +1018,7 @@
         fa.progress = pipe ? b->d_progress.as<uint32_t>() : nullptr;
         fa.n_strip_items = pipe ? (uint32_t)n_strip_items : 0u;
         fa.err_host = (uint32_t *)ctx->h_err.dp;
-        fa.pad3 = 0;
+        fa.all_fast = pr.all_fast && !fa.n_strip_items && !n_col_items ? 1u : 0u;
         if (attempt == 0) b->timing.col_chunks += (uint32_t)n_col_items + (pipe ? (uint32_t)pr.n_strip_chunks : 0u);
         fa.col_items = n_col_items ? b->d_col_items.as<ColItem>() : nullptr;
         fa.n_col_items = (uint32_t)n_col_items;
diff --git a/sparksmithwaterman_amd/csrc/swmi_device.h b/sparksmithwaterman_amd/csrc/swmi_device.h
--- a/sparksmithwaterman_amd/csrc/swmi_device.h
+++ b/sparksmithwaterman_amd/csrc/swmi_device.h
@@ -8,6 +8,7 @@
 #endif
 
 #define SWMI_SEQ_PAD_WORDS 24u
+#define SWMI_OH_FRONT      64u
 #define SWMI_RMAX          4
 #ifndef SWMI_CK_BLOCKS
 #define SWMI_CK_BLOCKS     2u
@@ -82,6 +83,7 @@
 
 struct FillArgs {
     const uint32_t *seqw;
+    const uint32_t *ohw;
     const SeqDesc  *refs;
     const SeqDesc  *reads;
     const PairDesc *pairs;
@@ -104,7 +106,7 @@
     const StripItem *strip_items;
     uint32_t       *progress;
     uint32_t        n_strip_items;
-    uint32_t        pad3;
+    uint32_t        all_fast;
     uint32_t       *err_host;
     const ColItem  *col_items;
     uint32_t        n_col_items;
diff --git a/sparksmithwaterman_amd/csrc/swmi_kernels.hip b/sparksmithwaterman_amd/csrc/swmi_kernels.hip
--- a/sparksmithwaterman_amd/csrc/swmi_kernels.hip
+++ b/sparksmithwaterman_amd/csrc/swmi_kernels.hip
@@ -584,9 +584,8 @@
 };
 
 template <int R>
-__device__ __forceinline__ void sweep_step_ref(const int (&hin)[R], int (&hout)[R], int (&hp)[R], const int (&q)[R],
-                                               const int rb, int &rbn, const uint32_t feed_code, const uint32_t gm,
-                                               int &lm, const bool in_range) {
+__device__ __forceinline__ void sweep_cells_ref(const int (&hin)[R], int (&hout)[R], int (&hp)[R], const int (&q)[R],
+                                                const int rb, const uint32_t gm, int &lm, const bool in_range) {
     const int nw = wave_shr1_zero(hout[R - 1]);
     const int upp = wave_shr1_zero(hp[R - 1]);
     if (in_range) {
@@ -606,6 +605,12 @@
 #pragma unroll
         for (int k = 0; k < R; ++k) hout[k] = hin[k];
     }
+}
+template <int R>
+__device__ __forceinline__ void sweep_step_ref(const int (&hin)[R], int (&hout)[R], int (&hp)[R], const int (&q)[R],
+                                               const int rb, int &rbn, const uint32_t feed_code, const uint32_t gm,
+                                               int &lm, const bool in_range) {
+    sweep_cells_ref<R>(hin, hout, hp, q, rb, gm, lm, in_range);
     rbn = wave_shr1((int)(1u << (feed_code & 31u)), rb);
 }
 
@@ -643,6 +648,31 @@
 #endif
 }
 
+__device__ __forceinline__ void load_oh16(uint32_t (&o)[16], const uint32_t *__restrict__ p) {
+#pragma unroll
+    for (int s = 0; s < 16; ++s) o[s] = p[s];
+}
+
+template <int R>
+__device__ __forceinline__ void sweep_tail_block_oh(SweepState<R> &S, const uint32_t (&o)[16], const uint32_t t0,
+                                                    const uint32_t lane_eff, const uint32_t n, const uint32_t gm) {
+#ifndef SWMI_NO_ASM
+    const uint32_t c = t0 - lane_eff;
+#pragma unroll
+    for (uint32_t s = 0; s < 16; s += 2) {
+        SweepStepTailOhAsm<R, 0>::run(S.h, S.g, S.hp, S.q, o[s], gm, S.lmax, c + s, n);
+        SweepStepTailOhAsm<R, 1>::run(S.h, S.g, S.hp, S.q, o[s + 1], gm, S.lmax, c + s + 1u, n);
+    }
+#else
+#pragma unroll
+    for (uint32_t s = 0; s < 16; ++s) {
+        const bool in_range = (t0 + s - lane_eff) < n;
+        if (s & 1u) sweep_cells_ref<R>(S.g, S.h, S.hp, S.q, (int)o[s], gm, S.lmax, in_range);
+        else        sweep_cells_ref<R>(S.h, S.g, S.hp, S.q, (int)o[s], gm, S.lmax, in_range);
+    }
+#endif
+}
+
 template <int R, bool COLS>
 __device__ __forceinline__ void sweep_fast(const FillArgs &A, const PairDesc pd, const uint32_t lane, const ColItem ci) {
     const SeqDesc rd = A.refs[pd.ref_id];
@@ -653,14 +683,12 @@
     const uint32_t g_lo = COLS ? ci.g_lo : 0u, g_hi = COLS ? ci.g_hi : G.n_ck;
     const bool last = g_hi >= G.n_ck;
     const uint32_t n = (last ? n_full : 16u * SWMI_CK_BLOCKS * g_hi) - col0;
-    const uint32_t *__restrict__ refw = A.seqw + rd.boff + (col0 >> 2);
     const uint32_t *__restrict__ readw = A.seqw + qd.boff;
     const uint32_t lact = m >= G.rps ? WAVE : (m + R - 1) / R;
     const uint32_t lane_eff = lane < lact ? lane : 0x40000000u;
     const uint32_t T = n + lact - 1;
     const uint32_t nblk = last ? (T + 15u) / 16u : n / 16u;
     const uint32_t gm = (uint32_t)(-(int64_t)A.gap);
-    const int one = 1;
     int pair_max = 0;
 
     const unsigned long long dbg_t0 = A.dbg ? __builtin_amdgcn_s_memtime() : 0ull;
@@ -671,10 +699,10 @@
         S.h[k] = 0; S.g[k] = 0; S.hp[k] = 0;
     }
     S.lmax = -1;
-    const uint4 *__restrict__ refq = reinterpret_cast<const uint4 *>(refw);
-    uint4 wnext = refq[0];
-    S.rby = 0;
-    S.rbx = wave_shr1((int)(1u << (wnext.x & 31u)), 0);
+    const uint32_t *__restrict__ ohp = A.ohw + SWMI_OH_FRONT + 4ull * rd.boff + col0 - lane;
+    uint32_t oa[16], ob[16];
+    load_oh16(oa, ohp);
+    uint32_t o_last = 0;
 
     uint32_t *__restrict__ wsp = A.dir + pd.dir_off + lane;
     auto close_window = [&](uint32_t g) {
@@ -683,9 +711,9 @@
         pair_max = pair_max > wm ? pair_max : wm;
         S.lmax = -1;
     };
-    for (uint32_t tb = 0; tb < nblk; ++tb) {
-        const uint4 w = wnext;
-        wnext = refq[tb + 1];
+    auto block = [&](const uint32_t tb, uint32_t (&o)[16], uint32_t (&onext)[16]) {
+        const uint32_t t0 = 16u * tb;
+        load_oh16(onext, ohp + t0 + 16u);
         const uint32_t tbg = tb + (col0 >> 4);
         if ((tbg % SWMI_CK_BLOCKS) == 0u) {
             const uint32_t g = tbg / SWMI_CK_BLOCKS;
@@ -697,21 +725,30 @@
 #pragma unroll
                 for (int k = 0; k < R; ++k) ck[k * WAVE] = (uint32_t)S.h[k];
                 ck[R * WAVE] = (uint32_t)wave_shr1_zero(S.g[R - 1]);
-                ck[(R + 1) * WAVE] = (uint32_t)S.rby;
-            }
-        }
-        const uint32_t t0 = 16u * tb;
+                ck[(R + 1) * WAVE] = o_last;
+            }
+        }
+        if (COLS && t0 < WAVE) {
+#pragma unroll
+            for (uint32_t s = 0; s < 16; ++s) o[s] = t0 + s >= lane ? o[s] : 0u;
+        }
 #ifndef SWMI_NO_ASM
         if (t0 + 15u < n) {
-            SweepStep4Asm<R>::run(S.h, S.g, S.hp, S.q, S.rbx, S.rby, w.x, w.y, one, gm, S.lmax);
-            SweepStep4Asm<R>::run(S.h, S.g, S.hp, S.q, S.rbx, S.rby, w.y, w.z, one, gm, S.lmax);
-            SweepStep4Asm<R>::run(S.h, S.g, S.hp, S.q, S.rbx, S.rby, w.z, w.w, one, gm, S.lmax);
-            SweepStep4Asm<R>::run(S.h, S.g, S.hp, S.q, S.rbx, S.rby, w.w, wnext.x, one, gm, S.lmax);
+            SweepStep4OhAsm<R>::run(S.h, S.g, S.hp, S.q, o[0], o[1], o[2], o[3], gm, S.lmax);
+            SweepStep4OhAsm<R>::run(S.h, S.g, S.hp, S.q, o[4], o[5], o[6], o[7], gm, S.lmax);
+            SweepStep4OhAsm<R>::run(S.h, S.g, S.hp, S.q, o[8], o[9], o[10], o[11], gm, S.lmax);
+            SweepStep4OhAsm<R>::run(S.h, S.g, S.hp, S.q, o[12], o[13], o[14], o[15], gm, S.lmax);
         } else
 #endif
         {
-            sweep_tail_block<R>(S, w, wnext.x, t0, lane_eff, n, one, gm);
-        }
+            sweep_tail_block_oh<R>(S, o, t0, lane_eff, n, gm);
+        }
+        o_last = o[15];
+    };
+    for (uint32_t tb = 0; tb < nblk; tb += 2u) {
+        block(tb, oa, ob);
+        if (tb + 1u >= nblk) break;
+        block(tb + 1u, ob, oa);
     }
     {
         const uint32_t gl = (nblk - 1u + (col0 >> 4)) / SWMI_CK_BLOCKS;
@@ -799,6 +836,17 @@
 
 extern "C" __global__ void __launch_bounds__(WAVE * FILL_WAVES) __attribute__((amdgpu_waves_per_eu(4, 4)))
 sw_sweep_winmax_kernel(const FillArgs A) { fill_entry<SWMI_MODE_WINMAX>(A); }
+
+extern "C" __global__ void __launch_bounds__(WAVE * FILL_WAVES) __attribute__((amdgpu_waves_per_eu(4, 4)))
+sw_sweep_fast_kernel(const FillArgs A) {
+    const uint32_t pair = blockIdx.x * FILL_WAVES + (threadIdx.x >> 6);
+    if (pair >= A.n_pairs) return;
+    const uint32_t lane = threadIdx.x & 63u;
+    if (pair == 0 && lane == 0 && A.hdr) { A.hdr->reserved = 0; A.hdr->pad = 0; }
+    if (pair == 0 && lane == 0 && A.q_reset) *A.q_reset = 0u;
+    const PairDesc pd = A.pairs[pair];
+    sweep_fast_dispatch<false>(A, pd, lane, A.reads[pd.read_id].len, ColItem{0u, 0u, 0u, 0u});
+}
 
 extern "C" __global__ void __launch_bounds__(WAVE * FILL_WAVES)
 sw_sweep_winmax_strips_kernel(const FillArgs A) {
@@ -1982,7 +2030,7 @@
 extern "C" hipError_t swmi_launch_fill(const FillArgs *a, hipStream_t st, hipEvent_t ev_start, hipEvent_t ev_stop) {
     if (a->n_pairs == 0) return hipSuccess;
     static const bool attrs = [] {
-        allow_big_lds(sw_fill_kernel); allow_big_lds(sw_fill_score_kernel); allow_big_lds(sw_sweep_winmax_kernel);
+        allow_big_lds(sw_fill_kernel); allow_big_lds(sw_fill_score_kernel); allow_big_lds(sw_sweep_winmax_kernel); allow_big_lds(sw_sweep_fast_kernel);
         allow_big_lds(sw_sweep_winmax_strips_kernel); allow_big_lds(sw_sweep_winmax_cols_kernel);
         return true;
     }();
@@ -1991,8 +2039,14 @@
     const size_t lds = spread_lds(grid.x);
     if (a->mode == 0)      hipLaunchKernelGGL(sw_fill_kernel, grid, block, lds, st, *a);
     else if (a->mode == 1) {
+        const bool fast = a->all_fast && !a->n_strip_items && !a->n_col_items;
         if (ev_start && ev_stop && !(a->skip_multi && a->n_strip_items) && !a->n_col_items) {
-            hipExtLaunchKernelGGL(sw_sweep_winmax_kernel, grid, block, (uint32_t)lds, st, ev_start, ev_stop, 0u, *a);
+            if (fast) hipExtLaunchKernelGGL(sw_sweep_fast_kernel, grid, block, (uint32_t)lds, st, ev_start, ev_stop, 0u, *a);
+            else      hipExtLaunchKernelGGL(sw_sweep_winmax_kernel, grid, block, (uint32_t)lds, st, ev_start, ev_stop, 0u, *a);
+            return hipGetLastError();
+        }
+        if (fast) {
+            hipLaunchKernelGGL(sw_sweep_fast_kernel, grid, block, lds, st, *a);
             return hipGetLastError();
         }
         hipLaunchKernelGGL(sw_sweep_winmax_kernel, grid, block, a->n_col_items || a->n_strip_items ? 0 : lds, st, *a);
diff --git a/sparksmithwaterman_amd/csrc/swmi_prep.hip b/sparksmithwaterman_amd/csrc/swmi_prep.hip
--- a/sparksmithwaterman_amd/csrc/swmi_prep.hip
+++ b/sparksmithwaterman_amd/csrc/swmi_prep.hip
@@ -7,7 +7,7 @@
 
 extern "C" __global__ void __launch_bounds__(WAVE * ENC_WAVES)
 sw_encode_kernel(const uint8_t *__restrict__ raw, const uint64_t *__restrict__ raw_off, SeqDesc *__restrict__ desc,
-                 uint32_t *__restrict__ seqw, const uint8_t *__restrict__ lut, uint32_t n_seq) {
+                 uint32_t *__restrict__ seqw, uint32_t *__restrict__ ohw, const uint8_t *__restrict__ lut, uint32_t n_seq) {
     __shared__ uint8_t T[256];
     T[threadIdx.x] = lut[threadIdx.x];
     __syncthreads();
@@ -17,6 +17,7 @@
     const uint64_t b0 = raw_off[s];
     const uint32_t len = (uint32_t)(raw_off[s + 1] - b0);
     uint32_t *__restrict__ img = seqw + desc[s].boff;
+    uint4 *__restrict__ oh = reinterpret_cast<uint4 *>(ohw + SWMI_OH_FRONT + 4ull * desc[s].boff);
     const uint8_t *__restrict__ src = raw + b0;
     const uint32_t nw = (len + 3u) >> 2;
     uint32_t bad = 0;
@@ -30,15 +31,17 @@
         v = c0 | (c1 << 8) | (c2 << 16) | (c3 << 24);
         bad |= v & 0xE3E3E3E3u;
         img[w] = v;
+        auto onehot = [&](uint32_t c, uint32_t k_) { return k_ < len && (c & 0xE3u) == 0u ? 1u << c : 0u; };
+        oh[w] = make_uint4(onehot(c0, k), onehot(c1, k + 1u), onehot(c2, k + 2u), onehot(c3, k + 3u));
     }
     const uint64_t anybad = __builtin_amdgcn_ballot_w64(bad != 0u);
     if (lane == 0) desc[s].acgt = anybad ? 0u : 1u;
 }
 
 extern "C" hipError_t swmi_launch_encode(const uint8_t *raw, const uint64_t *raw_off, SeqDesc *desc, uint32_t *seqw,
-                                         const uint8_t *lut, uint32_t n_seq, hipStream_t st) {
+                                         uint32_t *ohw, const uint8_t *lut, uint32_t n_seq, hipStream_t st) {
     if (n_seq == 0) return hipSuccess;
     hipLaunchKernelGGL(sw_encode_kernel, dim3((n_seq + ENC_WAVES - 1) / ENC_WAVES), dim3(WAVE * ENC_WAVES), 0, st,
-                       raw, raw_off, desc, seqw, lut, n_seq);
+                       raw, raw_off, desc, seqw, ohw, lut, n_seq);
     return hipGetLastError();
 }
diff --git a/sparksmithwaterman_amd/csrc/swmi_step_gen.inc b/sparksmithwaterman_amd/csrc/swmi_step_gen.inc
--- a/sparksmithwaterman_amd/csrc/swmi_step_gen.inc
+++ b/sparksmithwaterman_amd/csrc/swmi_step_gen.inc
@@ -698,6 +698,440 @@
             "v_cndmask_b32_e32 %[lm], %[lm], %[x], vcc\n\t"
             : [h0] "+v"(h[0]), [h1] "+v"(h[1]), [h2] "+v"(h[2]), [h3] "+v"(h[3]), [g0] "+v"(g[0]), [g1] "+v"(g[1]), [g2] "+v"(g[2]), [g3] "+v"(g[3]), [p0] "+v"(hp[0]), [p1] "+v"(hp[1]), [p2] "+v"(hp[2]), [p3] "+v"(hp[3]), [rbx] "+v"(rbx), [rby] "+v"(rby), [lm] "+v"(lm), [s0] "=&v"(s0), [a0] "=&v"(a0), [x] "=&v"(x), [a1] "=&v"(a1), [a2] "=&v"(a2), [a3] "=&v"(a3)
             : [q0] "v"(q[0]), [q1] "v"(q[1]), [q2] "v"(q[2]), [q3] "v"(q[3]), [wf0] "v"(wf0), [wf1] "v"(wf1), [one] "v"(one), [gm] "s"(gm), [c] "v"(c), [n] "v"(n)
+            : "vcc");
+    }
+};
+
+template <int R> struct SweepStep4OhAsm;
+
+template <> struct SweepStep4OhAsm<1> {
+    static __device__ __forceinline__ void run(int (&h)[1], int (&g)[1], int (&hp)[1], const int (&q)[1],
+                                               const uint32_t o0, const uint32_t o1, const uint32_t o2, const uint32_t o3,
+                                               const uint32_t gm, int &lm) {
+        int s0, a0, x;
+        asm volatile(
+            "v_dot8_i32_i4 %[s0], %[q0], %[o0], 0\n\t"
+            "v_max_i32_dpp %[x], %[p0], %[p0] wave_shr:1 row_mask:0xf bank_mask:0xf bound_ctrl:0\n\t"
+            "s_nop 1\n\t"
+            "v_add_u32_dpp %[a0], %[g0], %[s0] wave_shr:1 row_mask:0xf bank_mask:0xf bound_ctrl:0\n\t"
+            "v_max_i32_e32 %[g0], %[a0], %[x]\n\t"
+            "v_sub_u32_e64 %[p0], %[g0], %[gm] clamp\n\t"
+            "v_dot8_i32_i4 %[s0], %[q0], %[o1], 0\n\t"
+            "s_nop 0\n\t"
+            "v_max_i32_dpp %[x], %[p0], %[p0] wave_shr:1 row_mask:0xf bank_mask:0xf bound_ctrl:0\n\t"
+            "s_nop 0\n\t"
+            "v_add_u32_dpp %[a0], %[h0], %[s0] wave_shr:1 row_mask:0xf bank_mask:0xf bound_ctrl:0\n\t"
+            "v_max_i32_e32 %[h0], %[a0], %[x]\n\t"
+            "v_sub_u32_e64 %[p0], %[h0], %[gm] clamp\n\t"
+            "v_max3_i32 %[lm], %[lm], %[g0], %[h0]\n\t"
+            "v_dot8_i32_i4 %[s0], %[q0], %[o2], 0\n\t"
+            "v_max_i32_dpp %[x], %[p0], %[p0] wave_shr:1 row_mask:0xf bank_mask:0xf bound_ctrl:0\n\t"
+            "s_nop 1\n\t"
+            "v_add_u32_dpp %[a0], %[g0], %[s0] wave_shr:1 row_mask:0xf bank_mask:0xf bound_ctrl:0\n\t"
+            "v_max_i32_e32 %[g0], %[a0], %[x]\n\t"
+            "v_sub_u32_e64 %[p0], %[g0], %[gm] clamp\n\t"
+            "v_dot8_i32_i4 %[s0], %[q0], %[o3], 0\n\t"
+            "s_nop 0\n\t"
+            "v_max_i32_dpp %[x], %[p0], %[p0] wave_shr:1 row_mask:0xf bank_mask:0xf bound_ctrl:0\n\t"
+            "s_nop 0\n\t"
+            "v_add_u32_dpp %[a0], %[h0], %[s0] wave_shr:1 row_mask:0xf bank_mask:0xf bound_ctrl:0\n\t"
+            "v_max_i32_e32 %[h0], %[a0], %[x]\n\t"
+            "v_sub_u32_e64 %[p0], %[h0], %[gm] clamp\n\t"
+            "v_max3_i32 %[lm], %[lm], %[g0], %[h0]\n\t"
+            : [h0] "+v"(h[0]), [g0] "+v"(g[0]), [p0] "+v"(hp[0]), [lm] "+v"(lm), [s0] "=&v"(s0), [a0] "=&v"(a0), [x] "=&v"(x)
+            : [q0] "v"(q[0]), [o0] "v"(o0), [o1] "v"(o1), [o2] "v"(o2), [o3] "v"(o3), [gm] "s"(gm)
+            : );
+    }
+};
+
+template <> struct SweepStep4OhAsm<2> {
+    static __device__ __forceinline__ void run(int (&h)[2], int (&g)[2], int (&hp)[2], const int (&q)[2],
+                                               const uint32_t o0, const uint32_t o1, const uint32_t o2, const uint32_t o3,
+                                               const uint32_t gm, int &lm) {
+        int s0, a0, x, a1;
+        asm volatile(
+            "v_dot8_i32_i4 %[s0], %[q0], %[o0], 0\n\t"
+            "v_dot8c_i32_i4_e32 %[h0], %[q1], %[o0]\n\t"
+            "v_max_i32_dpp %[x], %[p1], %[p0] wave_shr:1 row_mask:0xf bank_mask:0xf bound_ctrl:0\n\t"
+            "s_nop 0\n\t"
+            "v_add_u32_dpp %[a0], %[g1], %[s0] wave_shr:1 row_mask:0xf bank_mask:0xf bound_ctrl:0\n\t"
+            "v_max_i32_e32 %[g0], %[a0], %[x]\n\t"
+            "v_sub_u32_e64 %[p0], %[g0], %[gm] clamp\n\t"
+            "v_max3_i32 %[g1], %[h0], %[p0], %[p1]\n\t"
+            "v_sub_u32_e64 %[p1], %[g1], %[gm] clamp\n\t"
+            "v_max3_i32 %[lm], %[lm], %[g0], %[g1]\n\t"
+            "v_dot8_i32_i4 %[s0], %[q0], %[o1], 0\n\t"
+            "v_dot8c_i32_i4_e32 %[g0], %[q1], %[o1]\n\t"
+            "v_max_i32_dpp %[x], %[p1], %[p0] wave_shr:1 row_mask:0xf bank_mask:0xf bound_ctrl:0\n\t"
+            "s_nop 0\n\t"
+            "v_add_u32_dpp %[a0], %[h1], %[s0] wave_shr:1 row_mask:0xf bank_mask:0xf bound_ctrl:0\n\t"
+            "v_max_i32_e32 %[h0], %[a0], %[x]\n\t"
+            "v_sub_u32_e64 %[p0], %[h0], %[gm] clamp\n\t"
+            "v_max3_i32 %[h1], %[g0], %[p0], %[p1]\n\t"
+            "v_sub_u32_e64 %[p1], %[h1], %[gm] clamp\n\t"
+            "v_max3_i32 %[lm], %[lm], %[h0], %[h1]\n\t"
+            "v_dot8_i32_i4 %[s0], %[q0], %[o2], 0\n\t"
+            "v_dot8c_i32_i4_e32 %[h0], %[q1], %[o2]\n\t"
+            "v_max_i32_dpp %[x], %[p1], %[p0] wave_shr:1 row_mask:0xf bank_mask:0xf bound_ctrl:0\n\t"
+            "s_nop 0\n\t"
+            "v_add_u32_dpp %[a0], %[g1], %[s0] wave_shr:1 row_mask:0xf bank_mask:0xf bound_ctrl:0\n\t"
+            "v_max_i32_e32 %[g0], %[a0], %[x]\n\t"
+            "v_sub_u32_e64 %[p0], %[g0], %[gm] clamp\n\t"
+            "v_max3_i32 %[g1], %[h0], %[p0], %[p1]\n\t"
+            "v_sub_u32_e64 %[p1], %[g1], %[gm] clamp\n\t"
+            "v_max3_i32 %[lm], %[lm], %[g0], %[g1]\n\t"
+            "v_dot8_i32_i4 %[s0], %[q0], %[o3], 0\n\t"
+            "v_dot8c_i32_i4_e32 %[g0], %[q1], %[o3]\n\t"
+            "v_max_i32_dpp %[x], %[p1], %[p0] wave_shr:1 row_mask:0xf bank_mask:0xf bound_ctrl:0\n\t"
+            "s_nop 0\n\t"
+            "v_add_u32_dpp %[a0], %[h1], %[s0] wave_shr:1 row_mask:0xf bank_mask:0xf bound_ctrl:0\n\t"
+            "v_max_i32_e32 %[h0], %[a0], %[x]\n\t"
+            "v_sub_u32_e64 %[p0], %[h0], %[gm] clamp\n\t"
+            "v_max3_i32 %[h1], %[g0], %[p0], %[p1]\n\t"
+            "v_sub_u32_e64 %[p1], %[h1], %[gm] clamp\n\t"
+            "v_max3_i32 %[lm], %[lm], %[h0], %[h1]\n\t"
+            : [h0] "+v"(h[0]), [h1] "+v"(h[1]), [g0] "+v"(g[0]), [g1] "+v"(g[1]), [p0] "+v"(hp[0]), [p1] "+v"(hp[1]), [lm] "+v"(lm), [s0] "=&v"(s0), [a0] "=&v"(a0), [x] "=&v"(x), [a1] "=&v"(a1)
+            : [q0] "v"(q[0]), [q1] "v"(q[1]), [o0] "v"(o0), [o1] "v"(o1), [o2] "v"(o2), [o3] "v"(o3), [gm] "s"(gm)
+            : );
+    }
+};
+
+template <> struct SweepStep4OhAsm<3> {
+    static __device__ __forceinline__ void run(int (&h)[3], int (&g)[3], int (&hp)[3], const int (&q)[3],
+                                               const uint32_t o0, const uint32_t o1, const uint32_t o2, const uint32_t o3,
+                                               const uint32_t gm, int &lm) {
+        int s0, a0, x, a1, a2;
+        asm volatile(
+            "v_dot8_i32_i4 %[s0], %[q0], %[o0], 0\n\t"
+            "v_dot8c_i32_i4_e32 %[h0], %[q1], %[o0]\n\t"
+            "v_dot8c_i32_i4_e32 %[h1], %[q2], %[o0]\n\t"
+            "v_max_i32_dpp %[x], %[p2], %[p0] wave_shr:1 row_mask:0xf bank_mask:0xf bound_ctrl:0\n\t"
+            "v_add_u32_dpp %[a0], %[g2], %[s0] wave_shr:1 row_mask:0xf bank_mask:0xf bound_ctrl:0\n\t"
+            "v_max_i32_e32 %[g0], %[a0], %[x]\n\t"
+            "v_sub_u32_e64 %[p0], %[g0], %[gm] clamp\n\t"
+            "v_max3_i32 %[g1], %[h0], %[p0], %[p1]\n\t"
+            "v_sub_u32_e64 %[p1], %[g1], %[gm] clamp\n\t"
+            "v_max3_i32 %[g2], %[h1], %[p1], %[p2]\n\t"
+            "v_sub_u32_e64 %[p2], %[g2], %[gm] clamp\n\t"
+            "v_max3_i32 %[lm], %[lm], %[g0], %[g1]\n\t"
+            "v_dot8_i32_i4 %[s0], %[q0], %[o1], 0\n\t"
+            "v_dot8c_i32_i4_e32 %[g0], %[q1], %[o1]\n\t"
+            "v_dot8c_i32_i4_e32 %[g1], %[q2], %[o1]\n\t"
+            "v_max_i32_dpp %[x], %[p2], %[p0] wave_shr:1 row_mask:0xf bank_mask:0xf bound_ctrl:0\n\t"
+            "v_add_u32_dpp %[a0], %[h2], %[s0] wave_shr:1 row_mask:0xf bank_mask:0xf bound_ctrl:0\n\t"
+            "v_max_i32_e32 %[h0], %[a0], %[x]\n\t"
+            "v_sub_u32_e64 %[p0], %[h0], %[gm] clamp\n\t"
+            "v_max3_i32 %[h1], %[g0], %[p0], %[p1]\n\t"
+            "v_sub_u32_e64 %[p1], %[h1], %[gm] clamp\n\t"
+            "v_max3_i32 %[h2], %[g1], %[p1], %[p2]\n\t"
+            "v_sub_u32_e64 %[p2], %[h2], %[gm] clamp\n\t"
+            "v_max3_i32 %[lm], %[lm], %[g2], %[h0]\n\t"
+            "v_max3_i32 %[lm], %[lm], %[h1], %[h2]\n\t"
+            "v_dot8_i32_i4 %[s0], %[q0], %[o2], 0\n\t"
+            "v_dot8c_i32_i4_e32 %[h0], %[q1], %[o2]\n\t"
+            "v_dot8c_i32_i4_e32 %[h1], %[q2], %[o2]\n\t"
+            "v_max_i32_dpp %[x], %[p2], %[p0] wave_shr:1 row_mask:0xf bank_mask:0xf bound_ctrl:0\n\t"
+            "v_add_u32_dpp %[a0], %[g2], %[s0] wave_shr:1 row_mask:0xf bank_mask:0xf bound_ctrl:0\n\t"
+            "v_max_i32_e32 %[g0], %[a0], %[x]\n\t"
+            "v_sub_u32_e64 %[p0], %[g0], %[gm] clamp\n\t"
+            "v_max3_i32 %[g1], %[h0], %[p0], %[p1]\n\t"
+            "v_sub_u32_e64 %[p1], %[g1], %[gm] clamp\n\t"
+            "v_max3_i32 %[g2], %[h1], %[p1], %[p2]\n\t"
+            "v_sub_u32_e64 %[p2], %[g2], %[gm] clamp\n\t"
+            "v_max3_i32 %[lm], %[lm], %[g0], %[g1]\n\t"
+            "v_dot8_i32_i4 %[s0], %[q0], %[o3], 0\n\t"
+            "v_dot8c_i32_i4_e32 %[g0], %[q1], %[o3]\n\t"
+            "v_dot8c_i32_i4_e32 %[g1], %[q2], %[o3]\n\t"
+            "v_max_i32_dpp %[x], %[p2], %[p0] wave_shr:1 row_mask:0xf bank_mask:0xf bound_ctrl:0\n\t"
+            "v_add_u32_dpp %[a0], %[h2], %[s0] wave_shr:1 row_mask:0xf bank_mask:0xf bound_ctrl:0\n\t"
+            "v_max_i32_e32 %[h0], %[a0], %[x]\n\t"
+            "v_sub_u32_e64 %[p0], %[h0], %[gm] clamp\n\t"
+            "v_max3_i32 %[h1], %[g0], %[p0], %[p1]\n\t"
+            "v_sub_u32_e64 %[p1], %[h1], %[gm] clamp\n\t"
+            "v_max3_i32 %[h2], %[g1], %[p1], %[p2]\n\t"
+            "v_sub_u32_e64 %[p2], %[h2], %[gm] clamp\n\t"
+            "v_max3_i32 %[lm], %[lm], %[g2], %[h0]\n\t"
+            "v_max3_i32 %[lm], %[lm], %[h1], %[h2]\n\t"
+            : [h0] "+v"(h[0]), [h1] "+v"(h[1]), [h2] "+v"(h[2]), [g0] "+v"(g[0]), [g1] "+v"(g[1]), [g2] "+v"(g[2]), [p0] "+v"(hp[0]), [p1] "+v"(hp[1]), [p2] "+v"(hp[2]), [lm] "+v"(lm), [s0] "=&v"(s0), [a0] "=&v"(a0), [x] "=&v"(x), [a1] "=&v"(a1), [a2] "=&v"(a2)
+            : [q0] "v"(q[0]), [q1] "v"(q[1]), [q2] "v"(q[2]), [o0] "v"(o0), [o1] "v"(o1), [o2] "v"(o2), [o3] "v"(o3), [gm] "s"(gm)
+            : );
+    }
+};
+
+template <> struct SweepStep4OhAsm<4> {
+    static __device__ __forceinline__ void run(int (&h)[4], int (&g)[4], int (&hp)[4], const int (&q)[4],
+                                               const uint32_t o0, const uint32_t o1, const uint32_t o2, const uint32_t o3,
+                                               const uint32_t gm, int &lm) {
+        int s0, a0, x, a1, a2, a3;
+        asm volatile(
+            "v_dot8_i32_i4 %[s0], %[q0], %[o0], 0\n\t"
+            "v_dot8c_i32_i4_e32 %[h0], %[q1], %[o0]\n\t"
+            "v_dot8c_i32_i4_e32 %[h1], %[q2], %[o0]\n\t"
+            "v_dot8c_i32_i4_e32 %[h2], %[q3], %[o0]\n\t"
+            "v_max_i32_dpp %[x], %[p3], %[p0] wave_shr:1 row_mask:0xf bank_mask:0xf bound_ctrl:0\n\t"
+            "v_add_u32_dpp %[a0], %[g3], %[s0] wave_shr:1 row_mask:0xf bank_mask:0xf bound_ctrl:0\n\t"
+            "v_max_i32_e32 %[g0], %[a0], %[x]\n\t"
+            "v_sub_u32_e64 %[p0], %[g0], %[gm] clamp\n\t"
+            "v_max3_i32 %[g1], %[h0], %[p0], %[p1]\n\t"
+            "v_sub_u32_e64 %[p1], %[g1], %[gm] clamp\n\t"
+            "v_max3_i32 %[g2], %[h1], %[p1], %[p2]\n\t"
+            "v_sub_u32_e64 %[p2], %[g2], %[gm] clamp\n\t"
+            "v_max3_i32 %[g3], %[h2], %[p2], %[p3]\n\t"
+            "v_sub_u32_e64 %[p3], %[g3], %[gm] clamp\n\t"
+            "v_max3_i32 %[lm], %[lm], %[g0], %[g1]\n\t"
+            "v_max3_i32 %[lm], %[lm], %[g2], %[g3]\n\t"
+            "v_dot8_i32_i4 %[s0], %[q0], %[o1], 0\n\t"
+            "v_dot8c_i32_i4_e32 %[g0], %[q1], %[o1]\n\t"
+            "v_dot8c_i32_i4_e32 %[g1], %[q2], %[o1]\n\t"
+            "v_dot8c_i32_i4_e32 %[g2], %[q3], %[o1]\n\t"
+            "v_max_i32_dpp %[x], %[p3], %[p0] wave_shr:1 row_mask:0xf bank_mask:0xf bound_ctrl:0\n\t"
+            "v_add_u32_dpp %[a0], %[h3], %[s0] wave_shr:1 row_mask:0xf bank_mask:0xf bound_ctrl:0\n\t"
+            "v_max_i32_e32 %[h0], %[a0], %[x]\n\t"
+            "v_sub_u32_e64 %[p0], %[h0], %[gm] clamp\n\t"
+            "v_max3_i32 %[h1], %[g0], %[p0], %[p1]\n\t"
+            "v_sub_u32_e64 %[p1], %[h1], %[gm] clamp\n\t"
+            "v_max3_i32 %[h2], %[g1], %[p1], %[p2]\n\t"
+            "v_sub_u32_e64 %[p2], %[h2], %[gm] clamp\n\t"
+            "v_max3_i32 %[h3], %[g2], %[p2], %[p3]\n\t"
+            "v_sub_u32_e64 %[p3], %[h3], %[gm] clamp\n\t"
+            "v_max3_i32 %[lm], %[lm], %[h0], %[h1]\n\t"
+            "v_max3_i32 %[lm], %[lm], %[h2], %[h3]\n\t"
+            "v_dot8_i32_i4 %[s0], %[q0], %[o2], 0\n\t"
+            "v_dot8c_i32_i4_e32 %[h0], %[q1], %[o2]\n\t"
+            "v_dot8c_i32_i4_e32 %[h1], %[q2], %[o2]\n\t"
+            "v_dot8c_i32_i4_e32 %[h2], %[q3], %[o2]\n\t"
+            "v_max_i32_dpp %[x], %[p3], %[p0] wave_shr:1 row_mask:0xf bank_mask:0xf bound_ctrl:0\n\t"
+            "v_add_u32_dpp %[a0], %[g3], %[s0] wave_shr:1 row_mask:0xf bank_mask:0xf bound_ctrl:0\n\t"
+            "v_max_i32_e32 %[g0], %[a0], %[x]\n\t"
+            "v_sub_u32_e64 %[p0], %[g0], %[gm] clamp\n\t"
+            "v_max3_i32 %[g1], %[h0], %[p0], %[p1]\n\t"
+            "v_sub_u32_e64 %[p1], %[g1], %[gm] clamp\n\t"
+            "v_max3_i32 %[g2], %[h1], %[p1], %[p2]\n\t"
+            "v_sub_u32_e64 %[p2], %[g2], %[gm] clamp\n\t"
+            "v_max3_i32 %[g3], %[h2], %[p2], %[p3]\n\t"
+            "v_sub_u32_e64 %[p3], %[g3], %[gm] clamp\n\t"
+            "v_max3_i32 %[lm], %[lm], %[g0], %[g1]\n\t"
+            "v_max3_i32 %[lm], %[lm], %[g2], %[g3]\n\t"
+            "v_dot8_i32_i4 %[s0], %[q0], %[o3], 0\n\t"
+            "v_dot8c_i32_i4_e32 %[g0], %[q1], %[o3]\n\t"
+            "v_dot8c_i32_i4_e32 %[g1], %[q2], %[o3]\n\t"
+            "v_dot8c_i32_i4_e32 %[g2], %[q3], %[o3]\n\t"
+            "v_max_i32_dpp %[x], %[p3], %[p0] wave_shr:1 row_mask:0xf bank_mask:0xf bound_ctrl:0\n\t"
+            "v_add_u32_dpp %[a0], %[h3], %[s0] wave_shr:1 row_mask:0xf bank_mask:0xf bound_ctrl:0\n\t"
+            "v_max_i32_e32 %[h0], %[a0], %[x]\n\t"
+            "v_sub_u32_e64 %[p0], %[h0], %[gm] clamp\n\t"
+            "v_max3_i32 %[h1], %[g0], %[p0], %[p1]\n\t"
+            "v_sub_u32_e64 %[p1], %[h1], %[gm] clamp\n\t"
+            "v_max3_i32 %[h2], %[g1], %[p1], %[p2]\n\t"
+            "v_sub_u32_e64 %[p2], %[h2], %[gm] clamp\n\t"
+            "v_max3_i32 %[h3], %[g2], %[p2], %[p3]\n\t"
+            "v_sub_u32_e64 %[p3], %[h3], %[gm] clamp\n\t"
+            "v_max3_i32 %[lm], %[lm], %[h0], %[h1]\n\t"
+            "v_max3_i32 %[lm], %[lm], %[h2], %[h3]\n\t"
+            : [h0] "+v"(h[0]), [h1] "+v"(h[1]), [h2] "+v"(h[2]), [h3] "+v"(h[3]), [g0] "+v"(g[0]), [g1] "+v"(g[1]), [g2] "+v"(g[2]), [g3] "+v"(g[3]), [p0] "+v"(hp[0]), [p1] "+v"(hp[1]), [p2] "+v"(hp[2]), [p3] "+v"(hp[3]), [lm] "+v"(lm), [s0] "=&v"(s0), [a0] "=&v"(a0), [x] "=&v"(x), [a1] "=&v"(a1), [a2] "=&v"(a2), [a3] "=&v"(a3)
+            : [q0] "v"(q[0]), [q1] "v"(q[1]), [q2] "v"(q[2]), [q3] "v"(q[3]), [o0] "v"(o0), [o1] "v"(o1), [o2] "v"(o2), [o3] "v"(o3), [gm] "s"(gm)
+            : );
+    }
+};
+
+template <int R, int ODD> struct SweepStepTailOhAsm;
+
+template <> struct SweepStepTailOhAsm<1, 0> {
+    static __device__ __forceinline__ void run(int (&h)[1], int (&g)[1], int (&hp)[1], const int (&q)[1],
+                                               const uint32_t o, const uint32_t gm, int &lm, const uint32_t c, const uint32_t n) {
+        int s0, a0, x;
+        asm volatile(
+            "v_cmp_lt_u32_e32 vcc, %[c], %[n]\n\t"
+            "v_dot8_i32_i4 %[s0], %[q0], %[o], 0\n\t"
+            "v_max_i32_dpp %[x], %[p0], %[p0] wave_shr:1 row_mask:0xf bank_mask:0xf bound_ctrl:0\n\t"
+            "s_nop 1\n\t"
+            "v_add_u32_dpp %[a0], %[g0], %[s0] wave_shr:1 row_mask:0xf bank_mask:0xf bound_ctrl:0\n\t"
+            "v_max_i32_e32 %[g0], %[a0], %[x]\n\t"
+            "v_sub_u32_e64 %[p0], %[g0], %[gm] clamp\n\t"
+            "v_max3_i32 %[x], %[lm], %[g0], %[g0]\n\t"
+            "v_cndmask_b32_e32 %[lm], %[lm], %[x], vcc\n\t"
+            : [h0] "+v"(h[0]), [g0] "+v"(g[0]), [p0] "+v"(hp[0]), [lm] "+v"(lm), [s0] "=&v"(s0), [a0] "=&v"(a0), [x] "=&v"(x)
+            : [q0] "v"(q[0]), [o] "v"(o), [gm] "s"(gm), [c] "v"(c), [n] "v"(n)
+            : "vcc");
+    }
+};
+
+template <> struct SweepStepTailOhAsm<1, 1> {
+    static __device__ __forceinline__ void run(int (&h)[1], int (&g)[1], int (&hp)[1], const int (&q)[1],
+                                               const uint32_t o, const uint32_t gm, int &lm, const uint32_t c, const uint32_t n) {
+        int s0, a0, x;
+        asm volatile(
+            "v_cmp_lt_u32_e32 vcc, %[c], %[n]\n\t"
+            "v_dot8_i32_i4 %[s0], %[q0], %[o], 0\n\t"
+            "v_max_i32_dpp %[x], %[p0], %[p0] wave_shr:1 row_mask:0xf bank_mask:0xf bound_ctrl:0\n\t"
+            "s_nop 1\n\t"
+            "v_add_u32_dpp %[a0], %[h0], %[s0] wave_shr:1 row_mask:0xf bank_mask:0xf bound_ctrl:0\n\t"
+            "v_max_i32_e32 %[h0], %[a0], %[x]\n\t"
+            "v_sub_u32_e64 %[p0], %[h0], %[gm] clamp\n\t"
+            "v_max3_i32 %[x], %[lm], %[h0], %[h0]\n\t"
+            "v_cndmask_b32_e32 %[lm], %[lm], %[x], vcc\n\t"
+            : [h0] "+v"(h[0]), [g0] "+v"(g[0]), [p0] "+v"(hp[0]), [lm] "+v"(lm), [s0] "=&v"(s0), [a0] "=&v"(a0), [x] "=&v"(x)
+            : [q0] "v"(q[0]), [o] "v"(o), [gm] "s"(gm), [c] "v"(c), [n] "v"(n)
+            : "vcc");
+    }
+};
+
+template <> struct SweepStepTailOhAsm<2, 0> {
+    static __device__ __forceinline__ void run(int (&h)[2], int (&g)[2], int (&hp)[2], const int (&q)[2],
+                                               const uint32_t o, const uint32_t gm, int &lm, const uint32_t c, const uint32_t n) {
+        int s0, a0, x, a1;
+        asm volatile(
+            "v_cmp_lt_u32_e32 vcc, %[c], %[n]\n\t"
+            "v_dot8_i32_i4 %[s0], %[q0], %[o], 0\n\t"
+            "v_dot8c_i32_i4_e32 %[h0], %[q1], %[o]\n\t"
+            "v_max_i32_dpp %[x], %[p1], %[p0] wave_shr:1 row_mask:0xf bank_mask:0xf bound_ctrl:0\n\t"
+            "s_nop 0\n\t"
+            "v_add_u32_dpp %[a0], %[g1], %[s0] wave_shr:1 row_mask:0xf bank_mask:0xf bound_ctrl:0\n\t"
+            "v_max_i32_e32 %[g0], %[a0], %[x]\n\t"
+            "v_sub_u32_e64 %[p0], %[g0], %[gm] clamp\n\t"
+            "v_max3_i32 %[g1], %[h0], %[p0], %[p1]\n\t"
+            "v_sub_u32_e64 %[p1], %[g1], %[gm] clamp\n\t"
+            "v_max3_i32 %[x], %[lm], %[g0], %[g1]\n\t"
+            "v_cndmask_b32_e32 %[lm], %[lm], %[x], vcc\n\t"
+            : [h0] "+v"(h[0]), [h1] "+v"(h[1]), [g0] "+v"(g[0]), [g1] "+v"(g[1]), [p0] "+v"(hp[0]), [p1] "+v"(hp[1]), [lm] "+v"(lm), [s0] "=&v"(s0), [a0] "=&v"(a0), [x] "=&v"(x), [a1] "=&v"(a1)
+            : [q0] "v"(q[0]), [q1] "v"(q[1]), [o] "v"(o), [gm] "s"(gm), [c] "v"(c), [n] "v"(n)
+            : "vcc");
+    }
+};
+
+template <> struct SweepStepTailOhAsm<2, 1> {
+    static __device__ __forceinline__ void run(int (&h)[2], int (&g)[2], int (&hp)[2], const int (&q)[2],
+                                               const uint32_t o, const uint32_t gm, int &lm, const uint32_t c, const uint32_t n) {
+        int s0, a0, x, a1;
+        asm volatile(
+            "v_cmp_lt_u32_e32 vcc, %[c], %[n]\n\t"
+            "v_dot8_i32_i4 %[s0], %[q0], %[o], 0\n\t"
+            "v_dot8c_i32_i4_e32 %[g0], %[q1], %[o]\n\t"
+            "v_max_i32_dpp %[x], %[p1], %[p0] wave_shr:1 row_mask:0xf bank_mask:0xf bound_ctrl:0\n\t"
+            "s_nop 0\n\t"
+            "v_add_u32_dpp %[a0], %[h1], %[s0] wave_shr:1 row_mask:0xf bank_mask:0xf bound_ctrl:0\n\t"
+            "v_max_i32_e32 %[h0], %[a0], %[x]\n\t"
+            "v_sub_u32_e64 %[p0], %[h0], %[gm] clamp\n\t"
+            "v_max3_i32 %[h1], %[g0], %[p0], %[p1]\n\t"
+            "v_sub_u32_e64 %[p1], %[h1], %[gm] clamp\n\t"
+            "v_max3_i32 %[x], %[lm], %[h0], %[h1]\n\t"
+            "v_cndmask_b32_e32 %[lm], %[lm], %[x], vcc\n\t"
+            : [h0] "+v"(h[0]), [h1] "+v"(h[1]), [g0] "+v"(g[0]), [g1] "+v"(g[1]), [p0] "+v"(hp[0]), [p1] "+v"(hp[1]), [lm] "+v"(lm), [s0] "=&v"(s0), [a0] "=&v"(a0), [x] "=&v"(x), [a1] "=&v"(a1)
+            : [q0] "v"(q[0]), [q1] "v"(q[1]), [o] "v"(o), [gm] "s"(gm), [c] "v"(c), [n] "v"(n)
+            : "vcc");
+    }
+};
+
+template <> struct SweepStepTailOhAsm<3, 0> {
+    static __device__ __forceinline__ void run(int (&h)[3], int (&g)[3], int (&hp)[3], const int (&q)[3],
+                                               const uint32_t o, const uint32_t gm, int &lm, const uint32_t c, const uint32_t n) {
+        int s0, a0, x, a1, a2;
+        asm volatile(
+            "v_cmp_lt_u32_e32 vcc, %[c], %[n]\n\t"
+            "v_dot8_i32_i4 %[s0], %[q0], %[o], 0\n\t"
+            "v_dot8c_i32_i4_e32 %[h0], %[q1], %[o]\n\t"
+            "v_dot8c_i32_i4_e32 %[h1], %[q2], %[o]\n\t"
+            "v_max_i32_dpp %[x], %[p2], %[p0] wave_shr:1 row_mask:0xf bank_mask:0xf bound_ctrl:0\n\t"
+            "v_add_u32_dpp %[a0], %[g2], %[s0] wave_shr:1 row_mask:0xf bank_mask:0xf bound_ctrl:0\n\t"
+            "v_max_i32_e32 %[g0], %[a0], %[x]\n\t"
+            "v_sub_u32_e64 %[p0], %[g0], %[gm] clamp\n\t"
+            "v_max3_i32 %[g1], %[h0], %[p0], %[p1]\n\t"
+            "v_sub_u32_e64 %[p1], %[g1], %[gm] clamp\n\t"
+            "v_max3_i32 %[g2], %[h1], %[p1], %[p2]\n\t"
+            "v_sub_u32_e64 %[p2], %[g2], %[gm] clamp\n\t"
+            "v_max3_i32 %[x], %[lm], %[g0], %[g1]\n\t"
+            "v_cndmask_b32_e32 %[lm], %[lm], %[x], vcc\n\t"
+            "v_max3_i32 %[x], %[lm], %[g2], %[g2]\n\t"
+            "v_cndmask_b32_e32 %[lm], %[lm], %[x], vcc\n\t"
+            : [h0] "+v"(h[0]), [h1] "+v"(h[1]), [h2] "+v"(h[2]), [g0] "+v"(g[0]), [g1] "+v"(g[1]), [g2] "+v"(g[2]), [p0] "+v"(hp[0]), [p1] "+v"(hp[1]), [p2] "+v"(hp[2]), [lm] "+v"(lm), [s0] "=&v"(s0), [a0] "=&v"(a0), [x] "=&v"(x), [a1] "=&v"(a1), [a2] "=&v"(a2)
+            : [q0] "v"(q[0]), [q1] "v"(q[1]), [q2] "v"(q[2]), [o] "v"(o), [gm] "s"(gm), [c] "v"(c), [n] "v"(n)
+            : "vcc");
+    }
+};
+
+template <> struct SweepStepTailOhAsm<3, 1> {
+    static __device__ __forceinline__ void run(int (&h)[3], int (&g)[3], int (&hp)[3], const int (&q)[3],
+                                               const uint32_t o, const uint32_t gm, int &lm, const uint32_t c, const uint32_t n) {
+        int s0, a0, x, a1, a2;
+        asm volatile(
+            "v_cmp_lt_u32_e32 vcc, %[c], %[n]\n\t"
+            "v_dot8_i32_i4 %[s0], %[q0], %[o], 0\n\t"
+            "v_dot8c_i32_i4_e32 %[g0], %[q1], %[o]\n\t"
+            "v_dot8c_i32_i4_e32 %[g1], %[q2], %[o]\n\t"
+            "v_max_i32_dpp %[x], %[p2], %[p0] wave_shr:1 row_mask:0xf bank_mask:0xf bound_ctrl:0\n\t"
+            "v_add_u32_dpp %[a0], %[h2], %[s0] wave_shr:1 row_mask:0xf bank_mask:0xf bound_ctrl:0\n\t"
+            "v_max_i32_e32 %[h0], %[a0], %[x]\n\t"
+            "v_sub_u32_e64 %[p0], %[h0], %[gm] clamp\n\t"
+            "v_max3_i32 %[h1], %[g0], %[p0], %[p1]\n\t"
+            "v_sub_u32_e64 %[p1], %[h1], %[gm] clamp\n\t"
+            "v_max3_i32 %[h2], %[g1], %[p1], %[p2]\n\t"
+            "v_sub_u32_e64 %[p2], %[h2], %[gm] clamp\n\t"
+            "v_max3_i32 %[x], %[lm], %[h0], %[h1]\n\t"
+            "v_cndmask_b32_e32 %[lm], %[lm], %[x], vcc\n\t"
+            "v_max3_i32 %[x], %[lm], %[h2], %[h2]\n\t"
+            "v_cndmask_b32_e32 %[lm], %[lm], %[x], vcc\n\t"
+            : [h0] "+v"(h[0]), [h1] "+v"(h[1]), [h2] "+v"(h[2]), [g0] "+v"(g[0]), [g1] "+v"(g[1]), [g2] "+v"(g[2]), [p0] "+v"(hp[0]), [p1] "+v"(hp[1]), [p2] "+v"(hp[2]), [lm] "+v"(lm), [s0] "=&v"(s0), [a0] "=&v"(a0), [x] "=&v"(x), [a1] "=&v"(a1), [a2] "=&v"(a2)
+            : [q0] "v"(q[0]), [q1] "v"(q[1]), [q2] "v"(q[2]), [o] "v"(o), [gm] "s"(gm), [c] "v"(c), [n] "v"(n)
+            : "vcc");
+    }
+};
+
+template <> struct SweepStepTailOhAsm<4, 0> {
+    static __device__ __forceinline__ void run(int (&h)[4], int (&g)[4], int (&hp)[4], const int (&q)[4],
+                                               const uint32_t o, const uint32_t gm, int &lm, const uint32_t c, const uint32_t n) {
+        int s0, a0, x, a1, a2, a3;
+        asm volatile(
+            "v_cmp_lt_u32_e32 vcc, %[c], %[n]\n\t"
+            "v_dot8_i32_i4 %[s0], %[q0], %[o], 0\n\t"
+            "v_dot8c_i32_i4_e32 %[h0], %[q1], %[o]\n\t"
+            "v_dot8c_i32_i4_e32 %[h1], %[q2], %[o]\n\t"
+            "v_dot8c_i32_i4_e32 %[h2], %[q3], %[o]\n\t"
+            "v_max_i32_dpp %[x], %[p3], %[p0] wave_shr:1 row_mask:0xf bank_mask:0xf bound_ctrl:0\n\t"
+            "v_add_u32_dpp %[a0], %[g3], %[s0] wave_shr:1 row_mask:0xf bank_mask:0xf bound_ctrl:0\n\t"
+            "v_max_i32_e32 %[g0], %[a0], %[x]\n\t"
+            "v_sub_u32_e64 %[p0], %[g0], %[gm] clamp\n\t"
+            "v_max3_i32 %[g1], %[h0], %[p0], %[p1]\n\t"
+            "v_sub_u32_e64 %[p1], %[g1], %[gm] clamp\n\t"
+            "v_max3_i32 %[g2], %[h1], %[p1], %[p2]\n\t"
+            "v_sub_u32_e64 %[p2], %[g2], %[gm] clamp\n\t"
+            "v_max3_i32 %[g3], %[h2], %[p2], %[p3]\n\t"
+            "v_sub_u32_e64 %[p3], %[g3], %[gm] clamp\n\t"
+            "v_max3_i32 %[x], %[lm], %[g0], %[g1]\n\t"
+            "v_cndmask_b32_e32 %[lm], %[lm], %[x], vcc\n\t"
+            "v_max3_i32 %[x], %[lm], %[g2], %[g3]\n\t"
+            "v_cndmask_b32_e32 %[lm], %[lm], %[x], vcc\n\t"
+            : [h0] "+v"(h[0]), [h1] "+v"(h[1]), [h2] "+v"(h[2]), [h3] "+v"(h[3]), [g0] "+v"(g[0]), [g1] "+v"(g[1]), [g2] "+v"(g[2]), [g3] "+v"(g[3]), [p0] "+v"(hp[0]), [p1] "+v"(hp[1]), [p2] "+v"(hp[2]), [p3] "+v"(hp[3]), [lm] "+v"(lm), [s0] "=&v"(s0), [a0] "=&v"(a0), [x] "=&v"(x), [a1] "=&v"(a1), [a2] "=&v"(a2), [a3] "=&v"(a3)
+            : [q0] "v"(q[0]), [q1] "v"(q[1]), [q2] "v"(q[2]), [q3] "v"(q[3]), [o] "v"(o), [gm] "s"(gm), [c] "v"(c), [n] "v"(n)
+            : "vcc");
+    }
+};
+
+template <> struct SweepStepTailOhAsm<4, 1> {
+    static __device__ __forceinline__ void run(int (&h)[4], int (&g)[4], int (&hp)[4], const int (&q)[4],
+                                               const uint32_t o, const uint32_t gm, int &lm, const uint32_t c, const uint32_t n) {
+        int s0, a0, x, a1, a2, a3;
+        asm volatile(
+            "v_cmp_lt_u32_e32 vcc, %[c], %[n]\n\t"
+            "v_dot8_i32_i4 %[s0], %[q0], %[o], 0\n\t"
+            "v_dot8c_i32_i4_e32 %[g0], %[q1], %[o]\n\t"
+            "v_dot8c_i32_i4_e32 %[g1], %[q2], %[o]\n\t"
+            "v_dot8c_i32_i4_e32 %[g2], %[q3], %[o]\n\t"
+            "v_max_i32_dpp %[x], %[p3], %[p0] wave_shr:1 row_mask:0xf bank_mask:0xf bound_ctrl:0\n\t"
+            "v_add_u32_dpp %[a0], %[h3], %[s0] wave_shr:1 row_mask:0xf bank_mask:0xf bound_ctrl:0\n\t"
+            "v_max_i32_e32 %[h0], %[a0], %[x]\n\t"
+            "v_sub_u32_e64 %[p0], %[h0], %[gm] clamp\n\t"
+            "v_max3_i32 %[h1], %[g0], %[p0], %[p1]\n\t"
+            "v_sub_u32_e64 %[p1], %[h1], %[gm] clamp\n\t"
+            "v_max3_i32 %[h2], %[g1], %[p1], %[p2]\n\t"
+            "v_sub_u32_e64 %[p2], %[h2], %[gm] clamp\n\t"
+            "v_max3_i32 %[h3], %[g2], %[p2], %[p3]\n\t"
+            "v_sub_u32_e64 %[p3], %[h3], %[gm] clamp\n\t"
+            "v_max3_i32 %[x], %[lm], %[h0], %[h1]\n\t"
+            "v_cndmask_b32_e32 %[lm], %[lm], %[x], vcc\n\t"
+            "v_max3_i32 %[x], %[lm], %[h2], %[h3]\n\t"
+            "v_cndmask_b32_e32 %[lm], %[lm], %[x], vcc\n\t"
+            : [h0] "+v"(h[0]), [h1] "+v"(h[1]), [h2] "+v"(h[2]), [h3] "+v"(h[3]), [g0] "+v"(g[0]), [g1] "+v"(g[1]), [g2] "+v"(g[2]), [g3] "+v"(g[3]), [p0] "+v"(hp[0]), [p1] "+v"(hp[1]), [p2] "+v"(hp[2]), [p3] "+v"(hp[3]), [lm] "+v"(lm), [s0] "=&v"(s0), [a0] "=&v"(a0), [x] "=&v"(x), [a1] "=&v"(a1), [a2] "=&v"(a2), [a3] "=&v"(a3)
+            : [q0] "v"(q[0]), [q1] "v"(q[1]), [q2] "v"(q[2]), [q3] "v"(q[3]), [o] "v"(o), [gm] "s"(gm), [c] "v"(c), [n] "v"(n)
             : "vcc");
     }
 };
```

After: 2456, median of 6. About the same (+1.9%).
